# RobustFieldAutonomyLab/DRL_graph_exploration

Hardware: AMD Instinct MI355X
Metric: env-steps/sec (256 parallel envs, ~64-node graphs) (higher is better)
Workload: dtype f64; 1 GPU; configs[1]: 256 envs/GPU, 40x40 map (V=1600), 100 landmarks, belief update at ~59-node graphs (P=37.0 poses, L=22.2 landmarks, M=188 factors) from a device snapshot; envs_per_gpu=256, map_size=40, num_landmarks=100, parallelism=env-sharded x1

## Files before the change

### drl_graph_exploration_amd/_lib.py

```python
import ctypes as C
import os

from .config import DrlgxConfig

_HERE = os.path.dirname(os.path.abspath(__file__))
_PATH = os.environ.get("DRLGX_LIB_DEV", os.path.join(_HERE, "libdrlgx.so"))
_lib = None

N_TIMERS = 8


class DrlgxError(RuntimeError):
    pass


class CsrCache(C.Structure):
    _fields_ = [(n, C.c_void_p) for n in ("deg", "selfw", "ax", "ptr_dst", "end_dst", "ptr_src", "end_src", "nbr_dst", "nbr_src", "wn_dst",
                                          "wn_src")]
    NODE_WORDS = dict(deg=1, selfw=1, ax=8, ptr_dst=1, end_dst=1, ptr_src=1, end_src=1)
    EDGE_WORDS = dict(nbr_dst=1, nbr_src=1, wn_dst=1, wn_src=1)


def lib_path():
    return _PATH


SYMBOLS = [
    "drlgx_create", "drlgx_destroy", "drlgx_set_stream", "drlgx_synchronize", "drlgx_strerror", "drlgx_last_error",
    "drlgx_status_host", "drlgx_status_fetch_host", "drlgx_reset_host", "drlgx_step", "drlgx_utility", "drlgx_uncertainty_em", "drlgx_explored", "drlgx_metrics", "drlgx_cov_array",
    "drlgx_stage_reset_host", "drlgx_stage_set_prior_information_host", "drlgx_stage_set_prior_pose_host", "drlgx_stage_move", "drlgx_stage_measure", "drlgx_stage_add_measurements", "drlgx_stage_optimize",
    "drlgx_stage_update_map", "drlgx_set_planner_parameter", "drlgx_set_fixed_landmarks_host", "drlgx_fm2_update", "drlgx_fm2_update_steps", "drlgx_em_cost", "drlgx_em_cost_steps", "drlgx_set_dubins_leaf_scoring", "drlgx_em_plan_leaves", "drlgx_og_cost", "drlgx_set_sampler_parameter", "drlgx_set_sampler_obstacles", "drlgx_set_dubins_library_host", "drlgx_dubins_library", "drlgx_set_dubins_prefilter", "drlgx_em_plan", "drlgx_rrt_plan", "drlgx_step_plan", "drlgx_step_plans", "drlgx_step_plans_traced",
    "drlgx_line_plan", "drlgx_lookahead", "drlgx_lookahead_bounded", "drlgx_graph_capacity", "drlgx_graph", "drlgx_get_counts_host", "drlgx_counts",
    "drlgx_get_poses_host", "drlgx_get_landmarks_host", "drlgx_get_cov_traces_host", "drlgx_vm_shape",
    "drlgx_get_virtual_map_host", "drlgx_get_ground_truth_host", "drlgx_get_adjacency_host", "drlgx_get_factors_host",
    "drlgx_get_landmark_order_host", "drlgx_snapshot", "drlgx_restore", "drlgx_timing_enable",
    "drlgx_timing_read_host", "drlgx_debug_phase_clocks_host", "drlgx_debug_gemm_tile_rows", "drlgx_debug_map_form", "drlgx_debug_map_compact_ok", "drlgx_debug_disc_cells_bound", "drlgx_inc_stats_host", "drlgx_gcn_workspace_bytes", "drlgx_gcn_forward", "drlgx_gcn_forward_batched", "drlgx_gcn_backward",
    "drlgx_replay_collate", "drlgx_replay_collate_pair", "drlgx_dqn_targets", "drlgx_dqn_loss_grad", "drlgx_dqn_arena_bytes", "drlgx_dqn_arena_views", "drlgx_dqn_prepare", "drlgx_dqn_forward_backward", "drlgx_replay_cache_csr", "drlgx_gcn_collate_csr", "drlgx_gcn_forward_prebuilt", "drlgx_adam_step", "drlgx_adam_step_scaled", "drlgx_normalise_rewards",
    "drlgx_segment_softmax", "drlgx_segment_softmax_backward", "drlgx_mean_pool", "drlgx_mean_pool_backward",
    "drlgx_ggnn_workspace_bytes", "drlgx_ggnn_forward", "drlgx_ggnn_backward",
    "drlgx_greedy_plans",
    "drlgx_set_env_obstacles", "drlgx_obstacle_flags", "drlgx_follow_plans",
    "drlgx_unet_workspace_bytes", "drlgx_unet_forward", "drlgx_unet_backward", "drlgx_unet_topk", "drlgx_unet_augment_filter", "drlgx_unet_kept_nodes",
]


def lib():
    global _lib
    if _lib is not None:
        return _lib
    import torch
    if not os.path.exists(_PATH):
        raise DrlgxError(
            "libdrlgx.so not found at %s — build it with `python -c 'import __graft_entry__ as g; g.build()'` "
            "(hipcc --offload-arch=gfx950); there is no CPU fallback." % _PATH)
    L = C.CDLL(_PATH)
    vp, ip, dp = C.c_void_p, C.POINTER(C.c_int32), C.POINTER(C.c_double)
    L.drlgx_create.argtypes = [C.POINTER(DrlgxConfig), C.c_int, C.c_int, C.c_int, C.POINTER(vp)]
    L.drlgx_destroy.argtypes = [vp]
    L.drlgx_set_stream.argtypes = [vp, vp]
    L.drlgx_synchronize.argtypes = [vp]
    L.drlgx_strerror.restype = C.c_char_p
    L.drlgx_strerror.argtypes = [C.c_int]
    L.drlgx_last_error.restype = C.c_char_p
    L.drlgx_last_error.argtypes = [vp]
    L.drlgx_status_host.argtypes = [vp]
    L.drlgx_status_fetch_host.argtypes = [vp, vp, C.c_size_t, vp]
    L.drlgx_reset_host.argtypes = [vp, C.c_int, ip, C.POINTER(C.c_uint32), dp]
    L.drlgx_step.argtypes = [vp, vp, vp]
    L.drlgx_step_plan.argtypes = [vp, vp, vp, C.c_int, C.c_int]
    L.drlgx_step_plans.argtypes = [vp, vp, vp, C.c_int, C.c_int]
    L.drlgx_step_plans_traced.argtypes = [vp, vp, vp, C.c_int, C.c_double, C.c_double, C.c_int, vp, vp]
    L.drlgx_greedy_plans.argtypes = [vp, C.c_int, vp, C.c_int] + [vp] * 5 + [C.c_int, C.c_int, vp, vp, vp]
    if os.environ.get("DRLGX_LIB_DEV") is None or hasattr(L, "drlgx_follow_plans"):
        L.drlgx_set_env_obstacles.argtypes = [vp, C.c_int]
        L.drlgx_obstacle_flags.argtypes = [vp, vp]
        L.drlgx_follow_plans.argtypes = [vp, vp, vp, vp, vp, C.c_int, dp, C.c_double, C.c_double, C.c_int, vp, vp, vp, vp]
    L.drlgx_stage_reset_host.argtypes =[vp, C.c_int, ip, C.POINTER(C.c_uint32), dp]
    L.drlgx_stage_set_prior_information_host.argtypes = [vp, C.c_int, dp]
    L.drlgx_stage_set_prior_pose_host.argtypes = [vp, C.c_int, dp]
    L.drlgx_stage_move.argtypes = [vp, vp, vp]
    L.drlgx_stage_measure.argtypes = [vp, vp, vp, vp, vp]
    L.drlgx_stage_add_measurements.argtypes = [vp, vp, vp, vp, vp]
    L.drlgx_stage_optimize.argtypes = [vp, vp]
    L.drlgx_stage_update_map.argtypes = [vp, vp, C.c_int]
    L.drlgx_set_planner_parameter.argtypes = [vp, C.c_double, C.c_double, C.c_double, C.c_double, C.c_double, C.c_int]
    L.drlgx_set_fixed_landmarks_host.argtypes = [vp, C.c_int, dp]
    L.drlgx_fm2_update.argtypes = [vp, C.c_int, vp, vp, vp, vp, C.c_int, vp]
    L.drlgx_em_cost.argtypes = [vp, C.c_int, vp, vp, vp, C.c_int, vp, vp, vp]
    if os.environ.get("DRLGX_LIB_DEV") is None or hasattr(L, "drlgx_em_cost_steps"):
        L.drlgx_fm2_update_steps.argtypes = [vp, C.c_int, vp, vp, vp, vp, vp, C.c_int, vp]
        L.drlgx_em_cost_steps.argtypes = [vp, C.c_int, vp, vp, vp, vp, vp, C.c_int, vp, vp, vp]
        L.drlgx_set_dubins_leaf_scoring.argtypes = [vp, C.c_int]
        L.drlgx_em_plan_leaves.argtypes = [vp, C.c_int, ip, ip, vp, vp, vp, vp, vp, vp]
    L.drlgx_og_cost.argtypes = [vp, C.c_int, vp, vp, vp, vp, vp, vp]
    L.drlgx_set_sampler_parameter.argtypes = [vp, C.c_double, C.c_double, C.c_int]
    L.drlgx_set_sampler_obstacles.argtypes = [vp, C.c_int]
    L.drlgx_set_dubins_library_host.argtypes = [vp, dp]
    L.drlgx_dubins_library.argtypes = [vp, C.c_int, ip, dp, dp, dp, ip]
    L.drlgx_set_dubins_prefilter.argtypes = [vp, C.c_int]
    L.drlgx_em_plan.argtypes = [vp, C.c_int, vp, vp, C.c_int, C.c_int] + [vp] * 8
    L.drlgx_rrt_plan.argtypes = [vp, C.c_int, vp, vp, vp, vp, C.c_int] + [vp] * 6
    L.drlgx_utility.argtypes = [vp, vp, vp]
    L.drlgx_uncertainty_em.argtypes = [vp, C.c_int, vp]
    L.drlgx_explored.argtypes = [vp, vp]
    L.drlgx_metrics.argtypes = [vp, C.c_double, vp]
    L.drlgx_cov_array.argtypes = [vp, vp, vp]
    L.drlgx_line_plan.argtypes = [vp, C.c_int, vp, vp, vp, vp]
    L.drlgx_lookahead.argtypes = [vp, C.c_int, vp, vp, vp, vp]
    L.drlgx_lookahead_bounded.argtypes = [vp, C.c_int, vp, vp, vp, C.c_int, vp]
    L.drlgx_graph_capacity.argtypes = [vp, ip, ip, ip]
    L.drlgx_graph.argtypes = [vp] + [vp] * 8
    L.drlgx_get_counts_host.argtypes = [vp, C.c_int, ip]
    L.drlgx_counts.argtypes = [vp, vp]
    L.drlgx_get_poses_host.argtypes = [vp, C.c_int, dp, dp]
    L.drlgx_get_landmarks_host.argtypes = [vp, C.c_int, ip, dp, dp]
    L.drlgx_get_cov_traces_host.argtypes = [vp, C.c_int, dp, dp]
    L.drlgx_vm_shape.argtypes = [vp, ip, ip]
    L.drlgx_get_virtual_map_host.argtypes = [vp, C.c_int, dp, dp, dp, C.POINTER(C.c_uint8)]
    L.drlgx_get_ground_truth_host.argtypes = [vp, C.c_int, dp, dp]
    L.drlgx_get_adjacency_host.argtypes = [vp, C.c_int, dp, dp]
    L.drlgx_get_factors_host.argtypes = [vp, C.c_int, ip, ip, dp, dp]
    L.drlgx_get_landmark_order_host.argtypes = [vp, ip]
    L.drlgx_snapshot.argtypes = [vp, C.c_int]
    L.drlgx_restore.argtypes = [vp, C.c_int]
    L.drlgx_timing_enable.argtypes = [vp, C.c_int]
    L.drlgx_timing_read_host.argtypes = [vp, dp, C.POINTER(C.c_int64)]
    L.drlgx_debug_phase_clocks_host.argtypes = [vp, C.c_int, C.POINTER(C.c_int64)]
    L.drlgx_debug_gemm_tile_rows.argtypes = [C.c_int, C.c_int, C.c_int, C.c_int]
    L.drlgx_debug_map_form.argtypes = [C.c_int]
    L.drlgx_debug_map_compact_ok.argtypes = [vp, C.c_int]
    L.drlgx_debug_disc_cells_bound.argtypes = [C.c_double]
    L.drlgx_inc_stats_host.argtypes = [vp, C.POINTER(C.c_int64), C.c_int]
    L.drlgx_gcn_workspace_bytes.restype = C.c_size_t
    L.drlgx_gcn_workspace_bytes.argtypes = [C.c_int, C.c_int, C.c_int, C.c_int]
    L.drlgx_gcn_forward.argtypes = [vp] + [C.c_int] * 5 + [vp] * 12
    L.drlgx_gcn_backward.argtypes = [vp] + [C.c_int] * 5 + [vp] * 15
    L.drlgx_ggnn_workspace_bytes.restype = C.c_size_t
    L.drlgx_ggnn_workspace_bytes.argtypes = [C.c_int] * 5
    L.drlgx_ggnn_forward.argtypes = [vp] + [C.c_int] * 6 + [vp] * 13 + [C.c_int, vp, vp, C.c_int]
    L.drlgx_ggnn_backward.argtypes = [vp] + [C.c_int] * 6 + [vp] * 17
    L.drlgx_unet_workspace_bytes.restype = C.c_size_t
    L.drlgx_unet_workspace_bytes.argtypes = [C.c_int] * 6 + [C.c_double, C.c_int]
    L.drlgx_unet_forward.argtypes = [vp] + [C.c_int] * 5 + [C.c_double, C.c_int] + [vp] * 3 + [C.POINTER(vp)] + [vp] * 3 + [C.c_size_t, C.c_int, vp, vp,
                                                                                                                       C.c_int]
    L.drlgx_unet_backward.argtypes = [vp] + [C.c_int] * 5 + [C.c_double, C.c_int] + [vp] * 3 + [C.POINTER(vp), vp, vp, C.POINTER(vp), vp, C.c_size_t,
                                                                                                C.c_int, C.c_int]
    L.drlgx_unet_kept_nodes.argtypes = [vp] + [C.c_int] * 4 + [C.c_double, C.c_int, vp, C.c_size_t, C.c_int, C.c_int, C.c_int, vp, C.POINTER(C.c_int)]
    L.drlgx_unet_topk.argtypes = [vp, C.c_int, C.c_int, vp, vp, C.c_double, vp, vp, vp, vp]
    L.drlgx_unet_augment_filter.argtypes = [vp, C.c_int, C.c_int, vp, vp, C.c_int, vp, vp, C.c_int, vp, vp, vp, C.c_int64, vp, vp, vp]
    L.drlgx_replay_collate.argtypes = [vp, C.c_int, vp, vp, C.c_int, vp, C.c_int64, vp, vp, vp, C.c_int64, vp, vp, vp, vp, vp, vp]
    L.drlgx_replay_collate_pair.argtypes = [vp, C.c_int, vp, vp, C.c_int, vp, C.c_int64, vp, vp, vp, C.c_int64, vp, vp, vp, vp, vp, vp, vp]
    L.drlgx_gcn_forward_batched.argtypes = [vp] + [C.c_int] * 5 + [vp] * 12 + [C.c_int, vp, vp, C.c_int]
    L.drlgx_dqn_targets.argtypes = [vp, C.c_int, vp, vp, vp, C.c_double, C.c_int64, vp, vp]
    L.drlgx_dqn_loss_grad.argtypes = [vp, C.c_int, vp, vp, vp, C.c_double, vp, vp]
    i64 = C.c_int64
    L.drlgx_dqn_arena_bytes.restype = C.c_size_t
    L.drlgx_dqn_arena_bytes.argtypes = [C.c_int, i64, i64, i64, C.c_int, C.c_int, C.c_int]
    L.drlgx_dqn_arena_views.argtypes = [vp, C.c_int, i64, i64, i64, C.c_int, C.c_int, C.c_int, C.POINTER(vp)]
    L.drlgx_dqn_prepare.argtypes = [vp, C.c_int, vp, vp, vp, C.c_int, vp, i64, vp, vp, i64, i64, i64, vp, vp, C.c_double, vp, i64, i64, i64,
                                    C.c_int, C.c_int, C.POINTER(CsrCache)]
    L.drlgx_dqn_forward_backward.argtypes = [vp, C.c_int, i64, i64, C.c_int, C.c_int, C.c_int, C.c_int, C.POINTER(vp), vp, C.c_double,
                                             C.POINTER(vp), vp, i64, i64, i64, C.c_int]
    L.drlgx_replay_cache_csr.argtypes = [vp, C.c_int, vp, vp, C.c_int, vp, C.c_int, vp, i64, vp, C.POINTER(CsrCache)]
    L.drlgx_gcn_collate_csr.argtypes = [vp, C.c_int, vp, C.POINTER(CsrCache), C.c_int, C.c_int, C.c_int, C.c_int, vp, vp, vp, vp, vp, vp]
    L.drlgx_gcn_forward_prebuilt.argtypes = [vp] + [C.c_int] * 5 + [vp] * 9
    L.drlgx_normalise_rewards.argtypes = [vp, C.c_int, vp, vp, vp, vp, vp]
    L.drlgx_segment_softmax.argtypes = [vp, C.c_int, vp, vp, vp, vp]
    L.drlgx_segment_softmax_backward.argtypes = [vp, C.c_int, vp, vp, vp, vp, vp]
    L.drlgx_mean_pool.argtypes = [vp, C.c_int, vp, vp, C.c_int, vp]
    L.drlgx_mean_pool_backward.argtypes = [vp, C.c_int, vp, vp, C.c_int, vp]
    L.drlgx_adam_step.argtypes = [vp, C.c_int, C.POINTER(vp), C.POINTER(vp), C.POINTER(vp), C.POINTER(vp), C.POINTER(C.c_int64),
                                  C.c_double, C.c_double, C.c_double, C.c_double, C.c_int64, C.c_double]
    L.drlgx_adam_step_scaled.argtypes = [vp, C.c_int, C.POINTER(vp), C.POINTER(vp), C.POINTER(vp), C.POINTER(vp), C.POINTER(C.c_int64),
                                  C.c_double, C.c_double, C.c_double, C.c_double, C.c_int64, C.c_double, C.c_double]
    _lib = L
    return L


def stream_ptr(device):
    import torch
    idx = device.index if isinstance(device, torch.device) else device
    if idx is None:
        idx = torch.cuda.current_device()
    return torch._C._cuda_getCurrentRawStream(idx)


def check(rc, handle=None):
    if rc != 0:
        L = lib()
        msg = L.drlgx_strerror(rc).decode()
        if handle is not None:
            extra = L.drlgx_last_error(handle).decode()
            if extra:
                msg += " (" + extra + ")"
        raise DrlgxError("drlgx error %d: %s" % (rc, msg))
```

### drl_graph_exploration_amd/csrc/drlgx_dev.h

```cpp
#pragma once
#include <hip/hip_runtime.h>
#include <stdint.h>

#include "../../include/drlgx.h"
#include "map_carve.h"

#define DRLGX_MT_N 624
#define DRLGX_MT_STRIDE 626
#define DRLGX_CNT_STRIDE 8
#define DRLGX_RED_STRIDE 8
#define DRLGX_PRIOR_STRIDE 16

enum { C_P = 0, C_L = 1, C_M = 2, C_STEP = 3, C_ISAM = 4, C_NEWP = 5, C_NEWL = 6, C_FLAG = 7 };
enum { R_UTR = 0, R_KNOWN = 1, R_EXPL = 2, R_UDET = 3, R_UWTR = 4, R_DIST = 5, R_OBS = 6, R_LATCH = 7 };

struct DrlgxState {
  drlgx_config cfg;
  int n_envs, n_inst, n_roll;
  int P_max, L_max, M_max, LG, V, Vu, rows, cols, A_max;
  int win;
  int disc_cells;
  int count_explored;
  double lo_free, lo_occ, lo_min, lo_max, occ_thresh;
  int bbox_noop;
// ... 13 lines not shown
  double *gt_lm;
  const double *fixed_lm;
  int n_fixed;
  int *parent;
  uint32_t *mt;
  double *nrm_saved;
  int *nrm_has;
  int *cnt;
  double *th_pose;
  double *d_pose;
  double *th_lm;
  double *d_lm;
  int *lm_key;
  int *key_slot;
  double *prior;
  double *odo;
  int *meas_pose;
  int *meas_lm;
  double *meas_br;
  double *est_pose;
  double *est_lm;
  double *pose_info;
  double *lm_info;
  double *pose_tr;
  double *lm_tr;
  double *vm_prob;
  double *vm_info;
  uint8_t *vm_upd;
  double *vm_tr;
  double *red;
  double *slam_ws;
  size_t slam_ws_stride;
  int *slam_iws;
  size_t slam_iws_stride;
  int *status;
  double *jc;
  size_t jc_stride;
  int jc_ld;
  double *jd;
  int *jc_meta;
  unsigned long long *inc_stats;
  long long *prof;
  int prof_block;
  const DrlgxState *self_dev;
};

typedef const __attribute__((address_space(4))) DrlgxState *DrlgxStateConst;
__device__ __forceinline__ void drlgx_warm_state(DrlgxStateConst Sp) {
  static_assert(sizeof(DrlgxState) <= 14 * 64, "drlgx_warm_state touches fourteen lines");
  const unsigned long long sp = reinterpret_cast<unsigned long long>(Sp);
  unsigned int w0, w1, w2, w3, w4, w5, w6, w7, w8, w9, w10, w11, w12, w13;
  asm volatile("s_load_dword %0, %14, 0x0\n\ts_load_dword %1, %14, 0x40\n\ts_load_dword %2, %14, 0x80\n\t"
               "s_load_dword %3, %14, 0xc0\n\ts_load_dword %4, %14, 0x100\n\ts_load_dword %5, %14, 0x140\n\t"
               "s_load_dword %6, %14, 0x180\n\ts_load_dword %7, %14, 0x1c0\n\ts_load_dword %8, %14, 0x200\n\t"
               "s_load_dword %9, %14, 0x240\n\ts_load_dword %10, %14, 0x280\n\ts_load_dword %11, %14, 0x2c0\n\t"
               "s_load_dword %12, %14, 0x300\n\ts_load_dword %13, %14, 0x340\n\t"
               "s_waitcnt lgkmcnt(0)"
               : "=s"(w0), "=s"(w1), "=s"(w2), "=s"(w3), "=s"(w4), "=s"(w5), "=s"(w6), "=s"(w7), "=s"(w8), "=s"(w9), "=s"(w10), "=s"(w11),
                 "=s"(w12), "=s"(w13)
               : "s"(sp));
}

#define DRLGX_KS_PARAM DrlgxStateConst S_
#define DRLGX_KS_REF (*(const DrlgxState *)S_)
#define DRLGX_KS_ARG(S) ((DrlgxStateConst)(S).self_dev)

#define DRLGX_PROF(S, slot)                                                        \
  do {                                                                             \
    if ((S).prof && threadIdx.x == 0 && blockIdx.x == (S).prof_block) (S).prof[slot] = wall_clock64(); \
  } while (0)

__device__ __forceinline__ int drlgx_bid() {
  int b = blockIdx.x;
  asm volatile("" : "+v"(b));
  return __builtin_amdgcn_readfirstlane(b);
}

__device__ __forceinline__ int drlgx_tid() {
  int t = threadIdx.x;
  asm volatile("" : "+v"(t));
  return t;
}

struct LaunchSel {
  int base;
  int n;
  const uint8_t *active;
  const int32_t *n_act;
  int act_idx;
  int map_last_only = 0;
  int pcap = 0;
  int skip_map = 0;
  const unsigned char *simlog = nullptr;
  size_t simlog_roll = 0;
  int simlog_act = 0;
  int vm_from = -1;
  __host__ __device__ __forceinline__ int cap(int P_max) const { return pcap > 0 && pcap < P_max ? pcap : P_max; }
  __device__ __forceinline__ bool map_on(int i) const {
    return !(map_last_only && n_act) || act_idx == n_act[i] - 1;
  }
  __device__ __forceinline__ bool on(int i) const {
    if (active && !active[i]) return false;
    if (n_act && act_idx >= n_act[i]) return false;
    return true;
  }
};

struct Pose {
  double x, y, c, s;
};
struct P2 {
  double x, y;
};

__device__ __forceinline__ void rot_from_cos_sin(double c, double s, double &oc, double &os) {
  if (fabs(c * c + s * s - 1.0) > 1e-9) {
    double n = sqrt(c * c + s * s);
    c /= n;
    s /= n;
  }
  oc = c;
  os = s;
}
__device__ __forceinline__ Pose make_pose(double x, double y, double th) { return Pose{x, y, cos(th), sin(th)}; }
__device__ __forceinline__ double theta_of(const Pose &p) { return atan2(p.s, p.c); }
__device__ __forceinline__ Pose compose(const Pose &a, const Pose &b) {
  Pose r;
  rot_from_cos_sin(a.c * b.c - a.s * b.s, a.s * b.c + a.c * b.s, r.c, r.s);
  r.x = a.x + (a.c * b.x - a.s * b.y);
  r.y = a.y + (a.s * b.x + a.c * b.y);
  return r;
}
__device__ __forceinline__ Pose between(const Pose &p1, const Pose &p2, double *H1) {
  double c = p1.c * p2.c + p1.s * p2.s, s = -p1.s * p2.c + p1.c * p2.s;
  Pose r;
  rot_from_cos_sin(c, s, r.c, r.s);
  double dx = p2.x - p1.x, dy = p2.y - p1.y;
  r.x = p1.c * dx + p1.s * dy;
  r.y = -p1.s * dx + p1.c * dy;
  if (H1) {
    double dt1 = -p2.s * dx + p2.c * dy;
    double dt2 = -p2.c * dx - p2.s * dy;
    H1[0] = -r.c; H1[1] = -r.s; H1[2] = dt1;
    H1[3] = r.s;  H1[4] = -r.c; H1[5] = dt2;
    H1[6] = 0;    H1[7] = 0;    H1[8] = -1;
  }
  return r;
}
__device__ __forceinline__ P2 transform_to(const Pose &p, const P2 &pt) {
  double dx = pt.x - p.x, dy = pt.y - p.y;
  return P2{p.c * dx + p.s * dy, -p.s * dx + p.c * dy};
}
__device__ __forceinline__ P2 transform_from(const Pose &p, const P2 &q) {
  return P2{p.c * q.x - p.s * q.y + p.x, p.s * q.x + p.c * q.y + p.y};
}
template <bool JAC>
__device__ __forceinline__ double bearing_of(const Pose &p, const P2 &pt, double *Hx, double *Hl) {
  P2 d = transform_to(p, pt);
  double d2 = d.x * d.x + d.y * d.y, n = sqrt(d2);
  if (fabs(n) > 1e-5) {
    if (JAC) {
      double a = -d.y / d2, b = d.x / d2;
      Hx[0] = a * -1.0;
      Hx[1] = b * -1.0;
      Hx[2] = a * d.y + b * -d.x;
      Hl[0] = a * p.c + b * -p.s;
// ... 295 lines not shown
    const double x = 2.0 * mt_canonical_words(mt_peek(s, w), mt_peek(s, w + 1)) - 1.0;
    const double y = 2.0 * mt_canonical_words(mt_peek(s, w + 2), mt_peek(s, w + 3)) - 1.0;
    const double r2 = x * x + y * y;
    const bool acc = !(r2 > 1.0 || r2 == 0.0);
    const unsigned long long m = __ballot(acc);
    const int rank = __popcll(m & ((1ull << lane) - 1ull));
    const int j = have + rank;
    const int i0 = offset + 2 * j;
    if (acc && j < Np && i0 + 1 >= skip) {
      const double mult = sqrt(-2 * log(r2) / r2);
      if (i0 >= skip) out[i0 - skip] = y * mult;
      out[i0 + 1 - skip] = x * mult;
    }
    const int A = __popcll(m);
    if (have + A >= Np) {
      const unsigned long long last = __ballot(acc && rank == Np - have - 1);
      const int t = __ffsll((long long)last) - 1;
      s.cons += 4u * (uint32_t)(t + 1);
      have = Np;
    } else {
      s.cons += 256u;
      have += A;
    }
  }
  wave_lds_sync();
  if (R & 1) {
    ns.saved = out[count - skip];
    ns.has = 1;
  }
}
__device__ inline double rng_normal(MtStream &s, NormalState &ns, double m, double sd, int lane) {
  return normal01(s, ns, lane) * sd + m;
}
__device__ inline double rng_uniform_real(MtStream &s, double lo, double hi, int lane) {
  return (hi - lo) * mt_canonical(s, lane) + lo;
}

inline void drlgx_ensure_lds_attr(bool (&done)[32], const void *const *fns, int n, int bytes) {
  int dev = 0;
  if (hipGetDevice(&dev) != hipSuccess || dev < 0 || dev >= 32) dev = 0;
  if (done[dev]) return;
  for (int i = 0; i < n; ++i) (void)hipFuncSetAttribute(fns[i], hipFuncAttributeMaxDynamicSharedMemorySize, bytes);
  done[dev] = true;
}

__host__ __device__ inline size_t drlgx_sim_lds_bytes(int LG, int P_max) {
  size_t b = (size_t)2 * DRLGX_MT_STRIDE * 4 + (size_t)(2 * LG + 2) * 8 + (size_t)LG * 4 + 16;
  b = ((b + 7) & ~(size_t)7) + (size_t)2 * LG * 8;
  if (P_max <= 64) b = b > kmap::MapCarve::pose_tables_bytes(P_max) + 32 ? b : kmap::MapCarve::pose_tables_bytes(P_max) + 32;
  return (b + 31) & ~(size_t)31;
}

struct DrlgxField;
enum DrlgxSimLaunch { DRLGX_SIM_RESET, DRLGX_SIM_STEP, DRLGX_SIM_STEP_OBS, DRLGX_SIM_STAGE, DRLGX_SIM_PRESIM };
constexpr size_t kSimLdsLimit = 64 * 1024;
size_t drlgx_sim_launch_lds(DrlgxSimLaunch which, int LG, int n_measure = 1, size_t *dyn_out = nullptr);
void drlgx_launch_reset(const DrlgxState &S, hipStream_t st, int n, const int32_t *env_ids_dev, const uint32_t *seeds_dev,
                        const double *start_dev, int first_measure = 1);
void drlgx_launch_sim_stage(const DrlgxState &S, hipStream_t st, LaunchSel sel, const double *odom, int mode, int32_t *keys,
                            double *br, int32_t *count);
void drlgx_launch_add_measurements(const DrlgxState &S, hipStream_t st, LaunchSel sel, const int32_t *keys, const double *br,
                                   const int32_t *count);
size_t drlgx_simlog_entry_bytes(const DrlgxState &S);
void drlgx_launch_presim(const DrlgxState &S, hipStream_t st, LaunchSel sel, const double *odom, int odom_stride, int n_measure, int a_end,
                         unsigned char *simlog, size_t simlog_roll, int simlog_act);
void drlgx_launch_sim(const DrlgxState &S, hipStream_t st, LaunchSel sel, const double *odom, int odom_stride,
                      int n_measure);
void drlgx_launch_sim_obs(const DrlgxState &S, hipStream_t st, LaunchSel sel, const double *odom, int odom_stride);
void drlgx_launch_slam(const DrlgxState &S, hipStream_t st, LaunchSel sel, int p_bound);
size_t drlgx_map_lds_bytes(const DrlgxState &S, int *chunk_out, int pcap = 0);
bool drlgx_step_fusable(const DrlgxState &S, int p_bound);
bool drlgx_step_arrow_fusable(const DrlgxState &S);
void drlgx_launch_step_arrow(const DrlgxState &S, hipStream_t st, LaunchSel sel, const double *odom, int odom_stride, int n_measure);
void drlgx_launch_step(const DrlgxState &S, hipStream_t st, LaunchSel sel, const double *odom, int odom_stride, int n_measure);
void drlgx_launch_step_loop(const DrlgxState &S, hipStream_t st, LaunchSel sel, const double *odom, int odom_stride, int n_measure, int a_end);
void drlgx_launch_step_arrow_loop(const DrlgxState &S, hipStream_t st, LaunchSel sel, const double *odom, int odom_stride, int n_measure, int a_end);
void drlgx_launch_map(const DrlgxState &S, hipStream_t st, LaunchSel sel, int rebuild);
bool drlgx_map_two_per_cu(const DrlgxState &S, int p_bound);
bool drlgx_map_compact_ok(const DrlgxState &S, int p_bound);
void drlgx_launch_copy(const DrlgxField *fields_dev, int n_fields, hipStream_t st, int n, const int32_t *src,
                       const int32_t *dst, int src_off, int dst_off, int skip_mask,
                       const int *cnt = nullptr,
                       const DrlgxState *panel = nullptr,
                       int only_cls = -1);
void drlgx_launch_rebase(const DrlgxState &S, hipStream_t st, int base0, int n);
inline size_t drlgx_fetch_head_bytes(int n_envs) { return ((size_t)(n_envs + 1) * sizeof(int) + 15) & ~(size_t)15; }
void drlgx_launch_fetch_pack(const DrlgxState &S, hipStream_t st, const void *src, size_t bytes, void *out);
void drlgx_launch_fix_rollouts(const DrlgxState &S, hipStream_t st, int n_cand, const int32_t *cand_env, int roll0);
void drlgx_launch_rewards(const DrlgxState &S, hipStream_t st, int n_cand, const int32_t *cand_env, int roll0,
                          double *rewards);
void drlgx_launch_utility(const DrlgxState &S, hipStream_t st, const double *dist, double *out, int mode);
void drlgx_launch_fm2_prior(const DrlgxState &S, hipStream_t st, const int32_t *env_ids, int n_env, double *sig, size_t sig_stride,
                            int n_max);
size_t drlgx_fm2_scratch_doubles(const DrlgxState &S, int nm_max);
void drlgx_launch_fm2_check(const DrlgxState &S, hipStream_t st, int n_cand, const int32_t *cand_env, const double *actions,
                            const int32_t *n_actions, const uint8_t *core, int nm_max, int *flag);
void drlgx_launch_fm2_update(const DrlgxState &S, hipStream_t st, int c0, int nc, const int32_t *cand_env, const int32_t *env_slot,
                             const double *actions, const int32_t *n_actions, const uint8_t *core, const double *sig, size_t sig_stride,
                             double *scratch, size_t scratch_stride, int *iscratch, int nm_max, double *cov_out, int out_stride,
                             int32_t *n_out);
size_t drlgx_em_lds_bytes(const DrlgxState &S);
void drlgx_launch_em_cost(const DrlgxState &S, hipStream_t st, int nc, const int32_t *cand_env, const double *actions,
                          const int32_t *n_actions, const uint8_t *core, const double *distance, const double *cov, int cov_stride,
                          int algorithm, double *unc_out, double *cost_out, double *info_out);
size_t drlgx_og_lds_bytes(const DrlgxState &S);
void drlgx_launch_og_check(const DrlgxState &S, hipStream_t st, int n_cand, const int32_t *cand_env, const int32_t *n_actions, int *flag);
void drlgx_launch_og_cost(const DrlgxState &S, hipStream_t st, int nc, const int32_t *cand_env, const double *actions,
                          const int32_t *n_actions, double *ent_out, double *cost_out, double *prob_out);
struct DrlgxDubins {
  const double *end_x, *end_y, *v, *w;
  const int *num_steps;
  int n, max_steps;
  double dt, tol, reach;
  double *pose;
};
struct DrlgxTreeArgs {
  int n_sel;
  const int32_t *env_sel;
  const int32_t *halton_start;
  int cap;
  int mode;
  double max_nodes;
  double safe_distance;
  const int32_t *goal_key;
  const double *goal_xy;
  double *act;
  int *link;
  int *leaf;
  int *meta;
  int *flag;
  double *nodes_out;
  int32_t *n_nodes_out, *result_out, *halton_next_out;
  DrlgxDubins lib;
};
size_t drlgx_em_tree_lds_bytes(int cap);
void drlgx_launch_em_tree(const DrlgxState &S, hipStream_t st, DrlgxTreeArgs args, bool obstacles, bool dubins);
void drlgx_launch_em_leaves_dubins(hipStream_t st, int n_sel, const int32_t *env_sel, int cap, int A_max, double angle_weight,
                                   const double *act, const int *link, const int *leaf, const int *meta, const DrlgxDubins &lib,
                                   int per_tree_row, int32_t *cand_env, double *actions, int32_t *n_actions, uint8_t *core,
                                   double *distance);
void drlgx_launch_em_leaves(hipStream_t st, int n_sel, const int32_t *env_sel, int cap, int A_max, const double *act, const int *link,
                            const int *leaf, const int *meta, int per_tree_row, int32_t *cand_env, double *actions, int32_t *n_actions);
void drlgx_launch_em_pick(hipStream_t st, int n_sel, int A_max, const int *meta, const double *cost, const double *actions,
                          const int32_t *n_actions, double *plan_out, int32_t *n_actions_out, double *cost_out, int32_t *n_leaves_out);
void drlgx_launch_metrics(const DrlgxState &S, hipStream_t st, double sigma0, double *out);
void drlgx_launch_plan_record(const DrlgxState &S, hipStream_t st, double sigma0, int a, int32_t *n_actions, double done_explored,
                              int max_steps, double *trace, int32_t *done);
void drlgx_launch_follow_select(const DrlgxState &S, hipStream_t st, const double *plan, const int32_t *n_actions, const int32_t *result,
                                const uint8_t *active, int steps, const double *fallback, double *act, int32_t *n_exec, int32_t *stop);
void drlgx_launch_follow_record(const DrlgxState &S, hipStream_t st, double sigma0, int a, const double *act, int32_t *n_exec, int obstacles,
                                double done_explored, int max_steps, double *trace, int32_t *done, int32_t *stop);
void drlgx_launch_obstacle_flags(const DrlgxState &S, hipStream_t st, uint8_t *out);
void drlgx_launch_cov_array(const DrlgxState &S, hipStream_t st, double *length, double *angle);
void drlgx_launch_line_plan(const DrlgxState &S, hipStream_t st, int n_cand, const int32_t *cand_env, const double *goal,
                            double *actions, int32_t *n_actions);
bool drlgx_slam_in_lds(int P_max, int L_max, int M_max);
bool drlgx_slam_capacity_ok(int P_max, int L_max, int M_max);
size_t drlgx_slam_ws_doubles(int P_max, int L_max, int M_max);
bool drlgx_graph_capacity_ok(int P_max, int L_max, int V);
void drlgx_launch_graph(const DrlgxState &S, hipStream_t st, int *gi, int gi_stride, int32_t *node_off, int32_t *edge_off,
                        float *x, int64_t *edge_index, float *edge_attr, int32_t *n_frontier, double *frontier_xy,
                        int32_t *nearest_node, int max_frontier);
```

### drl_graph_exploration_amd/csrc/drlgx_engine.cpp

```cpp
#include <hip/hip_runtime.h>

#include <algorithm>
#include <chrono>
#include <cmath>
#include <cstdio>
#include <cstring>
#include <functional>
#include <string>
#include <unordered_map>
#include <cstdlib>
#include <vector>

#include "drlgx_dev.h"
#include "drlgx_fields.h"

#define HIPCHK(e, call)                                                                       \
  do {                                                                                        \
    hipError_t _r = (call);                                                                   \
    if (_r != hipSuccess) {                                                                   \
      (e)->last_error = std::string(#call) + ": " + hipGetErrorString(_r);                    \
      return DRLGX_E_HIP;                                                                     \
    }                                                                                         \
  } while (0)

// ... 470 lines not shown
    std::unordered_map<unsigned, int> m;
    for (int i = 0; i < cfg->num_landmarks; ++i) m.emplace((unsigned)i, i);
    for (const auto &kv : m) e->lm_order.push_back((int)kv.first);
    if (e->lm_order.empty()) e->lm_order.push_back(0);
  }
  TRY(upload_table(e, &S.sweep_b, sweep));
  TRY(upload_table(e, &S.lm_order, e->lm_order));
  TRY(upload_table(e, &S.lo_pv, lo_pv));
  TRY(alloc_fields(e));
  S.slam_ws_stride = drlgx_slam_ws_doubles(S.P_max, S.L_max, S.M_max);
  S.slam_iws_stride = 2;
  TRY(dev_alloc(e, &S.slam_ws, S.slam_ws_stride * (size_t)S.n_inst));
  TRY(dev_alloc(e, &S.slam_iws, S.slam_iws_stride * (size_t)S.n_inst));
  TRY(alloc_panels(e));
  TRY(alloc_staging(e));
  HIPCHK(e, hipStreamSynchronize(e->stream));
  return DRLGX_OK;
}
#undef TRY

extern "C" {

const char *drlgx_strerror(int code) {
  switch (code) {
    case DRLGX_OK: return "ok";
    case DRLGX_E_INVALID: return "invalid argument";
    case DRLGX_E_NODEVICE: return "no HIP device";
    case DRLGX_E_CAPACITY: return "instance capacity exceeded (max_poses / max_landmarks / max_factors / max_actions)";
    case DRLGX_E_HIP: return "HIP runtime error";
    case DRLGX_E_NUMERIC: return "indeterminate linear system in the SLAM solve";
    default: return "unknown error";
  }
}

const char *drlgx_last_error(const drlgx_engine *e) {
  if (e) return e->last_error.c_str();
  return g_create_error.empty() ? "null engine" : g_create_error.c_str();
}

int drlgx_create(const drlgx_config *cfg, int n_envs, int n_rollouts, int device, drlgx_engine **out) {
  if (!out) return DRLGX_E_INVALID;
  g_create_error.clear();
  int r = check_config(cfg, n_envs, n_rollouts);
  if (r) return r;
  int ndev = 0;
  if (hipGetDeviceCount(&ndev) != hipSuccess || ndev <= 0 || device < 0 || device >= ndev) return DRLGX_E_NODEVICE;
  drlgx_engine *e = new drlgx_engine();
  e->device = device;
  if (hipSetDevice(device) != hipSuccess) {
    delete e;
    return DRLGX_E_NODEVICE;
  }
  if (hipStreamCreateWithFlags(&e->own_stream, hipStreamNonBlocking) != hipSuccess) {
    delete e;
    return DRLGX_E_NODEVICE;
  }
  e->stream = e->own_stream;
  DrlgxState &S = e->S;
  S.cfg = *cfg;
  S.n_envs = n_envs;
  S.n_roll = n_rollouts;
  if ((r = build_engine(e)) != DRLGX_OK) {
    g_create_error = e->last_error;
    drlgx_destroy(e);
    return r;
  }
  state_sync(e);
  *out = e;
  return DRLGX_OK;
}

static void state_sync(drlgx_engine *e) {
  if (!e->state_dev || memcmp(e->state_shadow, &e->S, sizeof(DrlgxState)) == 0) return;
  (void)hipStreamSynchronize(e->stream);
  (void)hipMemcpy(e->state_dev, &e->S, sizeof(DrlgxState), hipMemcpyHostToDevice);
  memcpy(e->state_shadow, &e->S, sizeof(DrlgxState));
}

static int snapshot_base(const drlgx_engine *e, int slot) { return 2 * e->S.n_envs + e->S.n_roll + slot * e->S.n_envs; }

static void settle(drlgx_engine *e) {
  if (e->owed_slot < 0) return;
  drlgx_launch_copy(e->fields_dev, (int)e->fields.size(), e->stream, e->S.n_envs, nullptr, nullptr, snapshot_base(e, e->owed_slot), 0, 0,
                    nullptr, nullptr, 1);
  e->owed_slot = -1;
}

int drlgx_destroy(drlgx_engine *e) {
  DRLGX_ENTER_OWING(e);
  if (!e) return DRLGX_E_INVALID;
  hipDeviceSynchronize();
  for (void *p : e->allocs) hipFree(p);
  for (auto &sp : e->spans) {
    hipEventDestroy(sp.a);
    hipEventDestroy(sp.b);
  }
  for (auto ev : e->free_events) hipEventDestroy(ev);
  if (e->sync_event) hipEventDestroy(e->sync_event);
  if (e->fetch_dev) hipFree(e->fetch_dev);
  if (e->fetch_host) hipHostFree(e->fetch_host);
  if (e->own_stream) hipStreamDestroy(e->own_stream);
  delete e;
  return DRLGX_OK;
}

int drlgx_set_stream(drlgx_engine *e, void *hip_stream) {
  DRLGX_ENTER_OWING(e);
  if (!e) return DRLGX_E_INVALID;
  hipStream_t s = (hip_stream == reinterpret_cast<void *>(-1)) ? e->own_stream : reinterpret_cast<hipStream_t>(hip_stream);
  if (s == e->stream) return DRLGX_OK;
  hipStreamSynchronize(e->stream);
  e->stream = s;
  return DRLGX_OK;
}

int drlgx_synchronize(drlgx_engine *e) {
  DRLGX_ENTER_OWING(e);
  if (!e) return DRLGX_E_INVALID;
  HIPCHK(e, hipStreamSynchronize(e->stream));
  return DRLGX_OK;
}

static int max_bound(const drlgx_engine *e) {
  if (e->by_capacity) return e->S.P_max;
  int m = 1;
  for (int v : e->pbound) m = std::max(m, v);
  return m;
}

static void advance_pbound(drlgx_engine *e, int k) {
  for (int &v : e->pbound) v = std::min(v + k, e->S.P_max);
}

static hipError_t stream_wait(drlgx_engine *e) {
  if (!e->spin_sync) return hipStreamSynchronize(e->stream);
  if (!e->sync_event && hipEventCreateWithFlags(&e->sync_event, hipEventDisableTiming) != hipSuccess) {
    (void)hipGetLastError();
    e->spin_sync = false;
    return hipStreamSynchronize(e->stream);
  }
  hipError_t r = hipEventRecord(e->sync_event, e->stream);
  if (r != hipSuccess) return r;
  const auto t0 = std::chrono::steady_clock::now();
  for (int polls = 0; (r = hipEventQuery(e->sync_event)) == hipErrorNotReady; ++polls) {
    if ((polls & 63) == 63 && std::chrono::steady_clock::now() - t0 > std::chrono::microseconds(5000)) return hipStreamSynchronize(e->stream);
  }
  return r;
}

static int status_fetch(drlgx_engine *e, const void *src_dev, size_t bytes, void *dst_host) {
  const size_t head = drlgx_fetch_head_bytes(e->S.n_envs), total = head + ((bytes + 15) & ~(size_t)15);
  if (total > e->fetch_cap) {
    HIPCHK(e, hipStreamSynchronize(e->stream));
    if (e->fetch_dev) (void)hipFree(e->fetch_dev);
    if (e->fetch_host) (void)hipHostFree(e->fetch_host);
    e->fetch_dev = e->fetch_host = nullptr;
    e->fetch_cap = 0;
    const size_t cap = std::max<size_t>(2 * total, 1 << 16);
    HIPCHK(e, hipMalloc(reinterpret_cast<void **>(&e->fetch_dev), cap));
    HIPCHK(e, hipHostMalloc(reinterpret_cast<void **>(&e->fetch_host), cap, hipHostMallocDefault));
    e->fetch_cap = cap;
  }
  drlgx_launch_fetch_pack(e->S, e->stream, src_dev, bytes, e->fetch_dev);
  HIPCHK(e, hipMemcpyAsync(e->fetch_host, e->fetch_dev, head + bytes, hipMemcpyDeviceToHost, e->stream));
  HIPCHK(e, stream_wait(e));
  const int32_t *h = reinterpret_cast<const int32_t *>(e->fetch_host);
  for (int i = 0; i < e->S.n_envs; ++i) e->pbound[i] = std::min(std::max((int)h[1 + i], 1), e->S.P_max);
// ... 998 lines not shown
  if (r) return r;
  const DrlgxState &S = e->S;
  const int L = c[1], M = c[2];
  std::vector<int> keys(L), mp(M), ml(M);
  std::vector<double> br((size_t)M * 2);
  if ((r = fetch(e, keys.data(), S.lm_key + (size_t)inst * S.L_max, (size_t)L * 4))) return r;
  if ((r = fetch(e, mp.data(), S.meas_pose + (size_t)inst * S.M_max, (size_t)M * 4))) return r;
  if ((r = fetch(e, ml.data(), S.meas_lm + (size_t)inst * S.M_max, (size_t)M * 4))) return r;
  if ((r = fetch(e, br.data(), S.meas_br + (size_t)inst * S.M_max * 2, (size_t)M * 16))) return r;
  HIPCHK(e, hipStreamSynchronize(e->stream));
  for (int m = 0; m < M; ++m) {
    if (pose) pose[m] = mp[m];
    if (key) key[m] = keys[ml[m]];
    if (bearing) bearing[m] = br[2 * m];
    if (range) range[m] = br[2 * m + 1];
  }
  return DRLGX_OK;
}

int drlgx_get_adjacency_host(drlgx_engine *e, int inst, double *adjacency, double *features) {
  DRLGX_ENTER(e);
  int32_t c[5];
  int r = drlgx_get_counts_host(e, inst, c);
  if (r) return r;
  const DrlgxState &S = e->S;
  const int P = c[0], L = c[1], M = c[2], N = P + L;
  std::vector<int> k, ord;
  if ((r = sorted_slots(e, inst, L, k, ord))) return r;
  std::vector<int> node_of_slot(L);
  for (int n = 0; n < L; ++n) node_of_slot[ord[n]] = n;
  std::vector<int> mp(M), ml(M);
  std::vector<double> br((size_t)M * 2), odo((size_t)P * 4), lt(L), pt(P);
  if ((r = fetch(e, mp.data(), S.meas_pose + (size_t)inst * S.M_max, (size_t)M * 4))) return r;
  if ((r = fetch(e, ml.data(), S.meas_lm + (size_t)inst * S.M_max, (size_t)M * 4))) return r;
  if ((r = fetch(e, br.data(), S.meas_br + (size_t)inst * S.M_max * 2, (size_t)M * 16))) return r;
  if ((r = fetch(e, odo.data(), S.odo + (size_t)inst * S.P_max * 4, (size_t)P * 32))) return r;
  if ((r = fetch(e, lt.data(), S.lm_tr + (size_t)inst * S.L_max, (size_t)L * 8))) return r;
  if ((r = fetch(e, pt.data(), S.pose_tr + (size_t)inst * S.P_max, (size_t)P * 8))) return r;
  HIPCHK(e, hipStreamSynchronize(e->stream));
  if (adjacency) std::fill(adjacency, adjacency + (size_t)N * N, 0.0);
  if (features) std::fill(features, features + N, 0.0);
  for (int i = 0; i + 1 < P; ++i) {
    double d = std::sqrt(std::pow(odo[4 * i], 2) + std::pow(odo[4 * i + 1], 2)) + 0.001;
    int a = L + i, b = L + i + 1;
    if (adjacency) adjacency[(size_t)a * N + b] = adjacency[(size_t)b * N + a] = d;
    if (features) {
      features[a] = pt[i];
      features[b] = pt[i + 1];
    }
  }
  for (int m = 0; m < M; ++m) {
    int a = L + mp[m], b = node_of_slot[ml[m]];
    if (adjacency) adjacency[(size_t)a * N + b] = adjacency[(size_t)b * N + a] = br[2 * m + 1];
    if (features) {
      features[a] = pt[mp[m]];
      features[b] = lt[ml[m]];
    }
  }
  return DRLGX_OK;
}

int drlgx_get_landmark_order_host(const drlgx_engine *e, int32_t *order) {
  if (!e || !order) return DRLGX_E_INVALID;
  for (int i = 0; i < e->S.cfg.num_landmarks; ++i) order[i] = e->lm_order[i];
  return DRLGX_OK;
}

int drlgx_snapshot(drlgx_engine *e, int slot) {
  DRLGX_ENTER(e);
  if (!e || slot < 0 || slot >= e->S.cfg.max_snapshots) return DRLGX_E_INVALID;
  const DrlgxState &S = e->S;
  ScopedTimer t(e, 3);
  drlgx_launch_copy(e->fields_dev, (int)e->fields.size(), e->stream, S.n_envs, nullptr, nullptr, 0, snapshot_base(e, slot), 0, e->S.cnt, &S);
  e->snap_pbound[slot] = e->pbound;
  return check_launch(e);
}

int drlgx_restore(drlgx_engine *e, int slot) {
  DRLGX_ENTER_OWING(e);
  if (!e || slot < 0 || slot >= e->S.cfg.max_snapshots) return DRLGX_E_INVALID;
  const DrlgxState &S = e->S;
  ScopedTimer t(e, 3);
  drlgx_launch_copy(e->fields_dev, (int)e->fields.size(), e->stream, S.n_envs, nullptr, nullptr, snapshot_base(e, slot), 0,
                    e->restore_eager ? 0 : 1, e->S.cnt, &S);
  e->owed_slot = e->restore_eager ? -1 : slot;
  e->pbound = e->snap_pbound[slot];
  return check_launch(e);
}

int drlgx_debug_phase_clocks_host(drlgx_engine *e, int arm, int64_t out[64]) {
  DRLGX_ENTER(e);
  if (!e) return DRLGX_E_INVALID;
  HIPCHK(e, hipStreamSynchronize(e->stream));
  e->S.prof_block = (arm >> 8) & 0xffff;
  if (out && e->S.prof)
    HIPCHK(e, hipMemcpy(out, e->S.prof + ((arm & 4) ? 0 : ((arm & 2) ? 64 : 0)), ((arm & 4) ? 1024 : 64) * sizeof(long long), hipMemcpyDeviceToHost));
  if (arm && !e->S.prof) {
    long long *p = nullptr;
    int r = dev_alloc(e, &p, 1024);
    if (r) return r;
    HIPCHK(e, hipStreamSynchronize(e->stream));
    e->S.prof = p;
  } else if (!arm) {
    e->S.prof = nullptr;
  }
  return DRLGX_OK;
}

int drlgx_inc_stats_host(drlgx_engine *e, int64_t out[2], int reset) {
  DRLGX_ENTER_OWING(e);
  if (!e || !out) return DRLGX_E_INVALID;
  out[0] = out[1] = -1;
  if (!e->S.inc_stats) return DRLGX_OK;
  unsigned long long v[2] = {0, 0};
  HIPCHK(e, hipMemcpyAsync(v, e->S.inc_stats, sizeof(v), hipMemcpyDeviceToHost, e->stream));
  if (reset) HIPCHK(e, hipMemsetAsync(e->S.inc_stats, 0, sizeof(v), e->stream));
  HIPCHK(e, hipStreamSynchronize(e->stream));
  out[0] = (int64_t)v[0];
  out[1] = (int64_t)v[1];
  return DRLGX_OK;
}

int drlgx_timing_enable(drlgx_engine *e, int on) {
  DRLGX_ENTER_OWING(e);
  if (!e) return DRLGX_E_INVALID;
  e->timing = on != 0;
  e->per_stage = on == 2;
  return DRLGX_OK;
}

int drlgx_timing_read_host(drlgx_engine *e, double ms[DRLGX_N_TIMERS], int64_t launches[DRLGX_N_TIMERS]) {
  DRLGX_ENTER_OWING(e);
  if (!e) return DRLGX_E_INVALID;
  HIPCHK(e, hipStreamSynchronize(e->stream));
  for (auto &sp : e->spans) {
    float t = 0;
    if (hipEventElapsedTime(&t, sp.a, sp.b) == hipSuccess && sp.id >= 0 && sp.id < DRLGX_N_TIMERS) {
      e->t_ms[sp.id] += t;
      e->t_n[sp.id] += 1;
    }
    e->free_events.push_back(sp.a);
    e->free_events.push_back(sp.b);
  }
  e->spans.clear();
  for (int i = 0; i < DRLGX_N_TIMERS; ++i) {
    if (ms) ms[i] = e->t_ms[i];
    if (launches) launches[i] = e->t_n[i];
    e->t_ms[i] = 0;
    e->t_n[i] = 0;
  }
  return DRLGX_OK;
}

}
```

### drl_graph_exploration_amd/csrc/k_inc.hip

```cpp

#pragma once
#include <type_traits>
#include "k_slam_common.hip"
namespace kslam {
#pragma clang fp contract(on)

constexpr int IYS = 18;
constexpr int INF = 64;
constexpr int kStreamKB = 512;
constexpr int ISNT = 4;

__device__ __forceinline__ int *inc_meta(const DrlgxState &S, int inst) { return S.jc_meta + (size_t)inst * 4; }

__device__ __forceinline__ bool inc_precheck(const DrlgxState &S, int inst, int P_after, int tid, int *scratch, int meta0 = -1, int meta1 = 0,
                                             int isam = 0) {
  if (!S.jc) return false;
  const int *meta = inc_meta(S, inst);
  const int *cnt = S.cnt + (size_t)inst * DRLGX_CNT_STRIDE;
  if (meta0 < 0) {
    meta0 = meta[0];
    meta1 = meta[1];
    isam = cnt[C_ISAM];
  }
  if (meta0 != 1 || meta1 + 1 != P_after || P_after < 2) return false;
// ... 22 lines not shown
    if constexpr (kDist == 16) {
      const auto p = __builtin_amdgcn_permlane16_swap(w[h], w[h], false, false);
      w[h] = ((threadIdx.x >> 4) & 1) ? p[0] : p[1];
    } else {
      const auto p = __builtin_amdgcn_permlane32_swap(w[h], w[h], false, false);
      w[h] = ((threadIdx.x >> 5) & 1) ? p[0] : p[1];
    }
  }
  return __longlong_as_double(((long long)w[1] << 32) | w[0]);
}

template <int kShift>
__device__ __forceinline__ double row_shr_f64(double v) {
  const long long b = __double_as_longlong(v);
  const int lo = __builtin_amdgcn_update_dpp(0, (int)b, 0x110 + kShift, 0xf, 0xf, true);
  const int hi = __builtin_amdgcn_update_dpp(0, (int)(b >> 32), 0x110 + kShift, 0xf, 0xf, true);
  return __longlong_as_double(((long long)hi << 32) | (unsigned int)lo);
}

constexpr int INEW = 12;
struct IncCtx {
  int inst, P, pn, pp, L0, M0, Lcap, n1, n1p, a0, ldw;
  int *fre, *fnew, *fslot, *ictl;
  double *fq, *recs, *gs, *vvec, *wks, *thp, *thl, *dl, *Dl, *Y, *Yh, *cwl;
  bool wide;
  int snt, yrows;
  double *yt, *wim, *jt, *svv;
};
__device__ __forceinline__ bool inc_plan(const DrlgxState &S, int inst, int P, int lds_bytes, size_t smem_off, IncCtx &x, bool &lds_panel, int pc,
                                         int L0_known = -1, int M0_known = -1) {
  extern __shared__ __attribute__((aligned(16))) unsigned char smem_raw[];
  const int *meta = inc_meta(S, inst);
  x.inst = inst; x.P = P; x.pn = P - 1; x.pp = P - 2;
  x.L0 = L0_known >= 0 ? L0_known : meta[2];
  x.M0 = L0_known >= 0 ? M0_known : meta[3];
  x.Lcap = min(S.L_max, x.L0 + INEW);
  x.n1 = 3 * P + 2 * x.L0; x.n1p = (x.n1 + 15) & ~15;
  x.a0 = 3 + 2 * x.L0;
  x.ldw = (3 + 2 * x.Lcap + 31) & ~31;
  const int ncap = max(3 * P + 2 * x.Lcap, x.n1p);
  size_t plan_off = drlgx_sim_lds_bytes(S.LG, pc);
  if ((3 * P + 1 + 15) / 16 > kDenseTiles && 2 * S.L_max + 1 > 16 * 8) plan_off = 0;
  if (smem_off > plan_off) plan_off = smem_off;
  size_t off = (smem_off + 15) & ~(size_t)15;
  const size_t off0 = off;
  auto take = [&](size_t bytes) { unsigned char *q = smem_raw + off; off += (bytes + 15) & ~(size_t)15; return q; };
  x.fre = reinterpret_cast<int *>(take(INF * 4));
  x.fnew = reinterpret_cast<int *>(take(INF * 4));
  x.fslot = reinterpret_cast<int *>(take(INF * 4));
  x.ictl = reinterpret_cast<int *>(take(16));
  x.fq = reinterpret_cast<double *>(take(32 * 8));
  x.recs = reinterpret_cast<double *>(take(INF * REC * 8));
  x.gs = reinterpret_cast<double *>(take(INEW * 12 * 8));
  x.vvec = reinterpret_cast<double *>(take(32 * 8));
  x.wks = reinterpret_cast<double *>(take(5 * 16 * IYS * 8));
  x.thp = reinterpret_cast<double *>(take((size_t)P * 4 * 8));
  x.thl = reinterpret_cast<double *>(take((size_t)x.Lcap * 2 * 8));
  x.dl = reinterpret_cast<double *>(take((size_t)ncap * 8));
  x.Dl = reinterpret_cast<double *>(take((size_t)P * 6 * 8));
  x.Y = reinterpret_cast<double *>(take((size_t)(x.n1p + 1) * IYS * 8));
  x.cwl = reinterpret_cast<double *>(smem_raw + off);
  const size_t fixed = ((plan_off + 15) & ~(size_t)15) + (off - off0);
  if (fixed > (size_t)lds_bytes) return false;
  lds_panel = fixed + (size_t)ncap * x.ldw * 8 <= (size_t)lds_bytes;
  const size_t pan = lds_panel ? (size_t)ncap * x.ldw * 8 : 0, yh = (size_t)(x.n1p + 1) * IYS * 8;
  x.Yh = x.cwl + pan / 8;
  x.wide = fixed + pan + yh <= (size_t)lds_bytes;
  x.snt = 0;
  if (!lds_panel && (3 * P + 1 + 15) / 16 > kDenseTiles) {
    x.yrows = x.a0 + 1;
    const size_t y_off = (size_t)(reinterpret_cast<unsigned char *>(x.Y) - smem_raw);
    const size_t avail = (size_t)lds_bytes - (((plan_off + 15) & ~(size_t)15) + (y_off - off0));
    for (int t = ISNT; t >= 1 && !x.snt; --t)
      if ((size_t)t * x.yrows * IYS * 8 + (size_t)max(0, t * t - 5) * 16 * IYS * 8 + (size_t)16 * t * 8 * 8 + 64 * 8 <= avail) x.snt = t;
    x.yt = x.Y;
    x.wim = x.yt + (size_t)x.snt * x.yrows * IYS;
    x.jt = x.wim + (size_t)max(0, x.snt * x.snt - 5) * 16 * IYS;
    x.svv = x.jt + (size_t)16 * x.snt * 8;
  }
  return true;
}

template <bool kLds, bool kSub>
__device__ __forceinline__ void inc_pre(const DrlgxState &S, const IncCtx &x, int tid, const double *odom3, SubBarrier sb) {
  const int ft = kSub ? tid - 64 : tid, fn = kSub ? kThreads - 64 : kThreads, lane = tid & 63;
  auto bar = [&]() {
    if constexpr (kSub) sb.sync(lane);
    else __syncthreads();
  };
  const int inst = x.inst, P = x.P, pn = x.pn, pp = x.pp, L0 = x.L0, n1 = x.n1, a0 = x.a0;
  double *gpan = S.jc + (size_t)inst * S.jc_stride;
  auto growp = [&](int q) -> double * { return gpan + (size_t)(q < 3 * P ? q : q + 3 * (S.P_max - P)) * S.jc_ld; };
  auto rowp = [&](int q) -> double * {
    if constexpr (kLds) return x.cwl + (size_t)q * x.ldw;
    else return gpan + (size_t)(q < 3 * P ? q : q + 3 * (S.P_max - P)) * S.jc_ld;
  };
  const double *th_pose = S.th_pose + (size_t)inst * S.P_max * 4;
  const double *th_lm = S.th_lm + (size_t)inst * S.L_max * 2;
  const double *d_pose = S.d_pose + (size_t)inst * S.P_max * 3;
  const double *d_lm = S.d_lm + (size_t)inst * S.L_max * 2;
  const double *jd = S.jd + (size_t)inst * S.P_max * 6;
  if (S.prof && blockIdx.x == S.prof_block && ft == 0) S.prof[0] = wall_clock64();
  if (ft < 4) x.ictl[ft] = 0;
  if (ft == fn - 1) {
    const double *t1 = th_pose + 4 * pp;
    Pose p1{t1[0], t1[1], t1[2], t1[3]}, p2, om;
    if constexpr (kSub) {
      om = make_pose(odom3[0], odom3[1], odom3[2]);
      const double *ep = S.est_pose + ((size_t)inst * S.P_max + pp) * 4;
      p2 = compose(Pose{ep[0], ep[1], ep[2], ep[3]}, om);
    } else {
      const double *t2 = th_pose + 4 * pn, *oo = S.odo + ((size_t)inst * S.P_max + pp) * 4;
      p2 = Pose{t2[0], t2[1], t2[2], t2[3]};
      om = Pose{oo[0], oo[1], oo[2], oo[3]};
    }
    double H1[9];
    const Pose hx = between(p1, p2, H1);
    const Pose h = between(om, hx, nullptr);
    const double e0 = h.x, e1 = h.y, e2 = theta_of(h);
    double *fq = x.fq;
    for (int k = 0; k < 9; ++k) fq[k] = -H1[k];
    fq[9] = -(h.c * e0 - h.s * e1);
    fq[10] = -(h.s * e0 + h.c * e1);
    fq[11] = -e2;
    x.thp[4 * pn] = p2.x; x.thp[4 * pn + 1] = p2.y; x.thp[4 * pn + 2] = p2.c; x.thp[4 * pn + 3] = p2.s;
  }
  for (int e = ft; e < 4 * pn; e += fn) x.thp[e] = th_pose[e];
  for (int e = ft; e < 2 * L0; e += fn) x.thl[e] = th_lm[e];
  for (int e = ft; e < 3 * pn; e += fn) x.dl[e] = d_pose[e];
  for (int e = ft; e < 2 * L0; e += fn) x.dl[3 * P + e] = d_lm[e];
  for (int e = ft; e < 6 * pn; e += fn) x.Dl[e] = jd[e];
  if constexpr (kLds) {
    const int npair = (a0 + 1) >> 1, nr = n1 - 3;
    const int cp0 = ft & 31, r0 = ft >> 5, rs = fn >> 5;
    for (int cp = cp0; cp < npair; cp += 32)
      for (int qq = r0; qq < nr; qq += 4 * rs) {
        const int q0 = qq, q1 = qq + rs, q2 = qq + 2 * rs, q3 = qq + 3 * rs;
        auto src = [&](int q) { const int c = min(q, nr - 1); return reinterpret_cast<const double2 *>(growp(c < 3 * pn ? c : c + 3))[cp]; };
        const double2 v0 = src(q0), v1 = src(q1), v2 = src(q2), v3 = src(q3);
        auto dst = [&](int q, const double2 &v) { if (q < nr) reinterpret_cast<double2 *>(rowp(q < 3 * pn ? q : q + 3))[cp] = v; };
        dst(q0, v0); dst(q1, v1); dst(q2, v2); dst(q3, v3);
      }
  }
  for (int e = ft; e < (x.n1p + 1 - n1) * IYS; e += fn) {
    x.Y[(size_t)n1 * IYS + e] = 0.0;
    if (x.wide) x.Yh[(size_t)n1 * IYS + e] = 0.0;
  }
  bar();
  if (S.prof && blockIdx.x == S.prof_block && ft == 0) S.prof[1] = wall_clock64();
  const double *fq = x.fq;
  {
    const double f00 = fq[0], f01 = fq[1], f02 = fq[2], f10 = fq[3], f11 = fq[4], f12 = fq[5], f20 = fq[6], f21 = fq[7], f22 = fq[8];
    for (int qq = ft; qq < n1 - 3; qq += fn) {
      const int q = qq < 3 * pn ? qq : qq + 3;
      double *r = rowp(q);
      const double t0 = r[0], t1 = r[1], t2 = r[2];
      r[0] = f00 * t0 + f01 * t1 + f02 * t2;
      r[1] = f10 * t0 + f11 * t1 + f12 * t2;
      r[2] = f20 * t0 + f21 * t1 + f22 * t2;
    }
  }
  bar();
  for (int e = ft; e < 3 * a0; e += fn) {
    const int r = e / a0, c = e - r * a0;
    double v = fq[3 * r] * rowp(3 * pp)[c] + fq[3 * r + 1] * rowp(3 * pp + 1)[c] + fq[3 * r + 2] * rowp(3 * pp + 2)[c];
    if (c == r) v += 1.0 / (c < 2 ? S.w_trans : S.w_rot);
    rowp(3 * pn + r)[c] = v;
  }
  if (ft < 3) x.dl[3 * pn + ft] = fq[3 * ft] * x.dl[3 * pp] + fq[3 * ft + 1] * x.dl[3 * pp + 1] + fq[3 * ft + 2] * x.dl[3 * pp + 2] + fq[9 + ft];
  if (S.prof && blockIdx.x == S.prof_block && ft == 0) S.prof[2] = wall_clock64();
}

template <bool kLds, int kSNT = ISNT>
__device__ __forceinline__ bool inc_post(const DrlgxState &S, const IncCtx &x, int L, int M, const SimBox &box, int tid,
                                         double *hand = nullptr, int hand_cap = 0) {
  const int lane = tid & 63, wave = tid >> 6, lc = lane & 15, lr = lane >> 4;
  const int inst = x.inst, P = x.P, pn = x.pn, L0 = x.L0, M0 = x.M0, n1 = x.n1, n1p = x.n1p, a0 = x.a0;
  int *meta = inc_meta(S, inst);
  const int nf = M - M0, nn = L - L0;
  const int n = 3 * P + 2 * L, a = 3 + 2 * L;
  int *fre = x.fre, *fnew = x.fnew, *fslot = x.fslot, *ictl = x.ictl;
  double *recs = x.recs, *gs = x.gs, *vvec = x.vvec, *wks = x.wks, *thp = x.thp, *thl = x.thl, *dl = x.dl, *Dl = x.Dl, *Y = x.Y;
  double *gpan = S.jc + (size_t)inst * S.jc_stride;
  auto growp = [&](int q) -> double * { return gpan + (size_t)(q < 3 * P ? q : q + 3 * (S.P_max - P)) * S.jc_ld; };
  auto rowp = [&](int q) -> double * {
    if constexpr (kLds) return x.cwl + (size_t)q * x.ldw;
    else return gpan + (size_t)(q < 3 * P ? q : q + 3 * (S.P_max - P)) * S.jc_ld;
  };
  int *cnt = S.cnt + (size_t)inst * DRLGX_CNT_STRIDE;
  double *d_pose = S.d_pose + (size_t)inst * S.P_max * 3;
  double *d_lm = S.d_lm + (size_t)inst * S.L_max * 2;
  double *jd = S.jd + (size_t)inst * S.P_max * 6;
  const bool feasible = nf >= 0 && nf <= INF && nn >= 0 && nn <= nf && L <= x.Lcap;
  const int *slot_src = box.br ? box.slot : S.meas_lm + (size_t)inst * S.M_max + M0;
  const double *br_src = box.br ? box.br : S.meas_br + ((size_t)inst * S.M_max + M0) * 2;
  const double *nl_src = box.br ? box.lm : S.th_lm + ((size_t)inst * S.L_max + L0) * 2;
  if (feasible && tid < 64) {
    const bool have = tid < nf;
    const int slot = have ? slot_src[tid] : -1;
    if (have) fslot[tid] = slot;
    bool bad = have && (slot < 0 || slot >= L);
    if (have && !box.br) bad |= S.meas_pose[(size_t)inst * S.M_max + M0 + tid] != pn;
    for (int t = 0; t < nf; ++t) {
      const int st = __builtin_amdgcn_readlane(slot, t);
      bad |= have && t < tid && st == slot;
    }
    const bool re = have && slot < L0, nw = have && slot >= L0;
    const unsigned long long mre = __ballot(re), mnw = __ballot(nw);
    if (re) fre[__popcll(mre & ((1ull << lane) - 1ull))] = tid;
    if (nw && !bad) fnew[slot - L0] = tid;
    if ((__ballot(bad) || __popcll(mnw) != nn) && lane == 0) ictl[2] = 1;
    if (lane == 0) ictl[0] = __popcll(mre);
  }
  for (int e = tid - 64; e >= 0 && e < 2 * nn && feasible; e += kThreads - 64) thl[2 * L0 + e] = nl_src[e];
  __syncthreads();
  if (!feasible || ictl[2]) {
    if (!kLds && tid == 0) meta[0] = 0;
    return false;
  }
  const int n_re = ictl[0];
  if (tid < nf) linearize_br(thp + 4 * pn, thl + 2 * fslot[tid], br_src[2 * tid], br_src[2 * tid + 1], recs + (size_t)REC * tid);
  __syncthreads();
  DRLGX_PROF(S, 35);
  const double Rb = S.cfg.bearing_noise * S.cfg.bearing_noise, Rr = S.cfg.range_noise * S.cfg.range_noise;
  const int ntr = n1p >> 4, ntc = (a0 + 15) >> 4;
  auto batch = [&](int b0, int nb, auto wide_tag) {
    constexpr bool kWide = decltype(wide_tag)::value;
    const int k = 2 * nb, kD = kWide ? k - 16 : 0;
    double *Yh = x.Yh;
    {
      constexpr int FS = kWide ? 16 : 8, RS = kThreads / FS;
      const int f = tid & (FS - 1);
      double j0 = 0, j1 = 0, j2 = 0, j3 = 0, j4 = 0, j5 = 0, l0c = 0, l1c = 0, l2c = 0, l3c = 0;
      int cl = 3;
      if (f < nb) {
        const int t = fre[b0 + f];
        const double *rc = recs + (size_t)REC * t;
        j0 = rc[0]; j1 = rc[1]; j2 = rc[2]; j3 = rc[3]; j4 = rc[4]; j5 = rc[5];
        l0c = rc[6]; l1c = rc[7]; l2c = rc[8]; l3c = rc[9];
        cl = 3 + 2 * fslot[t];
      }
      double *Yf = (kWide && f >= 8) ? Yh : Y;
      const int k0 = ks16(2 * (f & 7)), k1 = ks16(2 * (f & 7) + 1);
      for (int q0 = tid / FS; q0 < n1; q0 += 4 * RS) {
        double c0[4], c1[4], c2[4], l0[4], l1[4];
#pragma unroll
        for (int u = 0; u < 4; ++u) {
          const double *r = rowp(min(q0 + u * RS, n1 - 1));
          c0[u] = r[0]; c1[u] = r[1]; c2[u] = r[2]; l0[u] = r[cl]; l1[u] = r[cl + 1];
        }
#pragma unroll
        for (int u = 0; u < 4; ++u) {
          const int q = q0 + u * RS;
          if (q < n1) {
            Yf[(size_t)q * IYS + k0] = c0[u] * j0 + c1[u] * j1 + c2[u] * j2 + l0[u] * l0c + l1[u] * l1c;
            Yf[(size_t)q * IYS + k1] = c0[u] * j3 + c1[u] * j4 + c2[u] * j5 + l0[u] * l2c + l1[u] * l3c;
          }
        }
      }
    }
    __syncthreads();
    if (b0 == 0) DRLGX_PROF(S, 36);
    if (wave == 0) {
      auto tent = [&](int i, int j) -> double {
        const int t = fre[b0 + (i >> 1)], u = i & 1;
        const double *rc = recs + (size_t)REC * t;
        const double *Yj = (kWide && j >= 16) ? Yh : Y;
        const int col = ks16(j & 15);
        const double *yp = Yj + (size_t)(3 * pn) * IYS + col, *yl = Yj + (size_t)(3 * P + 2 * fslot[t]) * IYS + col;
        double sv = rc[3 * u] * yp[0] + rc[3 * u + 1] * yp[IYS] + rc[3 * u + 2] * yp[2 * IYS] + rc[6 + 2 * u] * yl[0] + rc[7 + 2 * u] * yl[IYS];
        if (i == j) sv += u ? Rr : Rb;
        return sv;
      };
      if (lane < (kWide ? 32 : 16)) {
        double v = 0.0;
        if (lane < k) {
          const int t = fre[b0 + (lane >> 1)], u = lane & 1;
          const double *rc = recs + (size_t)REC * t;
          const double *dp = dl + 3 * pn, *dq = dl + 3 * P + 2 * fslot[t];
          v = -rc[10 + u] - (rc[3 * u] * dp[0] + rc[3 * u + 1] * dp[1] + rc[3 * u + 2] * dp[2] + rc[6 + 2 * u] * dq[0] + rc[7 + 2 * u] * dq[1]);
        }
        vvec[(lane & 16) + ks16(lane & 15)] = v;
      }
      const int kA = kWide ? 16 : k;
      v4d d = {0.0, 0.0, 0.0, 0.0};
#pragma unroll
      for (int r = 0; r < 4; ++r) {
        const int i = lr + 4 * r, hi = max(i, lc), lo = min(i, lc);
        if (hi < kA) d[r] = tent(hi, lo);
      }
      const SweepCtx sx{0, lane, lc, lr, kA, 16, true, true, ictl + 1, nullptr};
      if constexpr (!kWide) {
        inv16_blk<true>(sx, kA, d);
        double *o = wks + lc * IYS + 4 * lr;
#pragma unroll
        for (int r = 0; r < 4; ++r) o[r] = (lc < k && lr + 4 * r < k) ? d[r] : 0.0;
      } else {
        v4d tb = {0.0, 0.0, 0.0, 0.0}, td = {0.0, 0.0, 0.0, 0.0};
#pragma unroll
        for (int r = 0; r < 4; ++r) {
          const int i = lr + 4 * r, hi = max(i, lc), lo = min(i, lc);
          if (lc < kD) tb[r] = tent(16 + lc, i);
          if (hi < kD) td[r] = tent(16 + hi, 16 + lo);
        }
        inv16_blk<false>(sx, 16, d);
        double a4[4] = {d[0], d[1], d[2], d[3]}, b4[4] = {tb[0], tb[1], tb[2], tb[3]};
        v4d xp = {0.0, 0.0, 0.0, 0.0};
        xp = mfma4(a4, b4, xp);
        double x4[4] = {xp[0], xp[1], xp[2], xp[3]};
        td = mfma4(b4, x4, td);
        const SweepCtx sd{0, lane, lc, lr, kD, 16, true, true, ictl + 1, nullptr};
        inv16_blk<true>(sd, kD, td);
        double *tsc = wks + 4 * 16 * IYS;
#pragma unroll
        for (int r = 0; r < 4; ++r) tsc[(lr + 4 * r) * IYS + ks16(lc)] = xp[r];
        wave_lds_sync();
        double xt4[4], s4[4];
        ld4(tsc + lc * IYS + 4 * lr, xt4);
#pragma unroll
        for (int r = 0; r < 4; ++r) s4[r] = (lc < kD && lr + 4 * r < kD) ? td[r] : 0.0;
        v4d w10 = {0.0, 0.0, 0.0, 0.0};
        w10 = mfma4(s4, xt4, w10);
        double w10a[4] = {w10[0], w10[1], w10[2], w10[3]};
        d = mfma4(w10a, xt4, d);
        double *o0 = wks + lc * IYS + 4 * lr, *o1 = o0 + 16 * IYS, *o3 = o0 + 3 * 16 * IYS;
#pragma unroll
        for (int r = 0; r < 4; ++r) {
          o0[r] = d[r];
          o1[r] = w10[r];
          o3[r] = s4[r];
          wks[2 * 16 * IYS + (lr + 4 * r) * IYS + ks16(lc)] = w10[r];
        }
      }
    }
    __syncthreads();
    if (b0 == 0) DRLGX_PROF(S, 37);
    if (wave < ntr) {
      const int npr = (a0 + 31) >> 5;
      const int nks = kWide ? 4 : (k + 3) >> 2;
      const int nks1 = kWide ? (kD + 3) >> 2 : 0;
      const int nun = ((ntr - wave + kWaves - 1) / kWaves) * npr;
      v4d aA0, aA1, aB0, aB1;
      double ua[4] = {0.0, 0.0, 0.0, 0.0}, ub[4] = {0.0, 0.0, 0.0, 0.0};
      auto loads = [&](int e, v4d &c0, v4d &c1) {
        const int it = e / npr, pr = e - it * npr, I = wave + kWaves * it;
#pragma unroll
        for (int r = 0; r < 4; ++r) {
          const double *rw = rowp(16 * I + lr + 4 * r) + 32 * pr + lc;
          c0[r] = rw[0];
          c1[r] = rw[16];
        }
      };
      auto unit = [&](int e, v4d &acc0, v4d &acc1) {
        const int it = e / npr, pr = e - it * npr, I = wave + kWaves * it;
        if (pr == 0) {
          double w4[4], yI[4], yH[4];
          ld4(wks + lc * IYS + 4 * lr, w4);
          ld4(Y + (size_t)(16 * I + lc) * IYS + 4 * lr, yI);
          v4d ut = {0.0, 0.0, 0.0, 0.0};
          ut = mfma4(w4, yI, ut);
          if constexpr (kWide) {
            ld4(Yh + (size_t)(16 * I + lc) * IYS + 4 * lr, yH);
            ld4(wks + 16 * IYS + lc * IYS + 4 * lr, w4);
            ut = mfma4(w4, yH, ut);
            v4d u2 = {0.0, 0.0, 0.0, 0.0};
            ld4(wks + 2 * 16 * IYS + lc * IYS + 4 * lr, w4);
            u2 = mfma4(w4, yI, u2);
            ld4(wks + 3 * 16 * IYS + lc * IYS + 4 * lr, w4);
            u2 = mfma4(w4, yH, u2);
            ub[0] = u2[0]; ub[1] = u2[1]; ub[2] = u2[2]; ub[3] = u2[3];
          }
          ua[0] = ut[0]; ua[1] = ut[1]; ua[2] = ut[2]; ua[3] = ut[3];
          const int q = 16 * I + lc;
          auto rowdot = [&](const double *vec, const double *vech) -> double {
            double y4[4];
            ld4(vec + 4 * lr, y4);
            double sdot = ua[0] * y4[0] + ua[1] * y4[1] + ua[2] * y4[2] + ua[3] * y4[3];
            if constexpr (kWide) {
              ld4(vech + 4 * lr, y4);
              sdot += ub[0] * y4[0] + ub[1] * y4[1] + ub[2] * y4[2] + ub[3] * y4[3];
            }
            sdot += rowgroup_xor<16>(sdot);
            sdot += rowgroup_xor<32>(sdot);
            return sdot;
          };
          const double sv = rowdot(vvec, vvec + 16);
          const bool prow = q < 3 * pn;
          const int qc = prow ? q : 0, pi = qc / 3, rp = qc - 3 * pi;
          const size_t o3 = (size_t)(3 * pi) * IYS;
          const double s0 = rowdot(Y + o3, Yh + o3), s1 = rowdot(Y + o3 + IYS, Yh + o3 + IYS), s2 = rowdot(Y + o3 + 2 * IYS, Yh + o3 + 2 * IYS);
          if (lr == 0 && q < n1) {
            dl[q] -= sv;
            if (prow) {
              double *D = Dl + 6 * pi + (rp * (rp + 1)) / 2;
              D[0] += s0;
              if (rp >= 1) D[1] += s1;
              if (rp >= 2) D[2] += s2;
            }
          }
        }
        {
          const int cA = 32 * pr + lc, cB = cA + 16;
          const int y0 = cA < 3 ? 3 * pn + cA : (cA < a0 ? 3 * P + cA - 3 : n1p);
          const int y1 = cB < a0 ? 3 * P + cB - 3 : n1p;
          double yJ0[4], yJ1[4];
          ld4(Y + (size_t)y0 * IYS + 4 * lr, yJ0);
          ld4(Y + (size_t)y1 * IYS + 4 * lr, yJ1);
#pragma unroll
          for (int ks = 0; ks < 4; ++ks)
            if (ks < nks) {
              acc0 = __builtin_amdgcn_mfma_f64_16x16x4f64(ua[ks], yJ0[ks], acc0, 0, 0, 0);
              acc1 = __builtin_amdgcn_mfma_f64_16x16x4f64(ua[ks], yJ1[ks], acc1, 0, 0, 0);
            }
          if constexpr (kWide) {
            ld4(Yh + (size_t)y0 * IYS + 4 * lr, yJ0);
            ld4(Yh + (size_t)y1 * IYS + 4 * lr, yJ1);
#pragma unroll
            for (int ks = 0; ks < 4; ++ks)
              if (ks < nks1) {
                acc0 = __builtin_amdgcn_mfma_f64_16x16x4f64(ub[ks], yJ0[ks], acc0, 0, 0, 0);
                acc1 = __builtin_amdgcn_mfma_f64_16x16x4f64(ub[ks], yJ1[ks], acc1, 0, 0, 0);
              }
          }
        }
#pragma unroll
        for (int r = 0; r < 4; ++r) {
          double *rw = rowp(16 * I + lr + 4 * r) + 32 * pr + lc;
          rw[0] = acc0[r];
          rw[16] = acc1[r];
        }
      };
      int e = 0;
      loads(0, aA0, aA1);
// ... 225 lines not shown
            }
          }
          sv += rowgroup_xor<16>(sv); sv += rowgroup_xor<32>(sv);
          so += rowgroup_xor<16>(so); so += rowgroup_xor<32>(so);
          s1 += rowgroup_xor<16>(s1); s1 += rowgroup_xor<32>(s1);
          s2 += rowgroup_xor<16>(s2); s2 += rowgroup_xor<32>(s2);
          if (lr == 0 && q >= 0) {
            dl[q] -= sv;
            if (q < 3 * pn) {
              const int pi = q / 3, rp = q - 3 * pi;
              double *D = Dl + 6 * pi + (rp * (rp + 1)) / 2;
              D[rp] += so;
              if (rp >= 1) D[rp - 1] += s1;
              if (rp >= 2) D[0] += s2;
            }
          }
        }
        {
          const int cA = min(32 * pr + lc, a0), cB = min(32 * pr + 16 + lc, a0);
#pragma unroll
          for (int mt = 0; mt < NT; ++mt) {
            double yJ0[4], yJ1[4];
            ld4(Yt + (size_t)mt * ytile + (size_t)cA * IYS + 4 * lr, yJ0);
            ld4(Yt + (size_t)mt * ytile + (size_t)cB * IYS + 4 * lr, yJ1);
#pragma unroll
            for (int ks = 0; ks < 4; ++ks)
              if (mt < NT - 1 || ks < nksl) {
                acc0 = __builtin_amdgcn_mfma_f64_16x16x4f64(ua[mt][ks], yJ0[ks], acc0, 0, 0, 0);
                acc1 = __builtin_amdgcn_mfma_f64_16x16x4f64(ua[mt][ks], yJ1[ks], acc1, 0, 0, 0);
              }
          }
        }
#pragma unroll
        for (int r = 0; r < 4; ++r) {
          const int q = rowq(I, lr + 4 * r);
          if (q >= 0) {
            double *rw = rowp(q) + 32 * pr + lc;
            rw[0] = acc0[r];
            rw[16] = acc1[r];
          }
        }
      };
      int e = 0;
      loads(0, aA0, aA1);
      for (; e + 1 < nun; e += 2) {
        loads(e + 1, aB0, aB1);
        unit(e, aA0, aA1);
        loads(min(e + 2, nun - 1), aA0, aA1);
        unit(e + 1, aB0, aB1);
      }
      if (e < nun) unit(e, aA0, aA1);
    }
    __syncthreads();
    if (b0 == 0) DRLGX_PROF(S, 38);
    else DRLGX_PROF(S, 47);
  };
  bool streamed = false;
  if constexpr (!kLds && kSNT > 0) {
    streamed = x.snt > 0 && (n_re > (x.wide ? 16 : 8) || (size_t)n1 * a0 * 8 > (size_t)(kStreamKB << 10));
  }
  if (streamed) {
    if constexpr (!kLds && kSNT > 0) {
      for (int b0 = 0; b0 < n_re;) {
        const int left = n_re - b0, nt = min(x.snt, (left + 7) >> 3), nb = min(8 * nt, left);
        if (nt >= 4) sbatch(b0, nb, std::integral_constant<int, kSNT >= 4 ? 4 : 1>{});
        else if (nt == 3) sbatch(b0, nb, std::integral_constant<int, 3>{});
        else if (nt == 2) sbatch(b0, nb, std::integral_constant<int, 2>{});
        else sbatch(b0, nb, std::integral_constant<int, 1>{});
        b0 += nb;
      }
    }
  } else {
    for (int b0 = 0; b0 < n_re;) {
      const int left = n_re - b0;
      if (left > 8 && x.wide) {
        const int nb = min(16, left);
        batch(b0, nb, std::true_type{});
        b0 += nb;
      } else {
        const int nb = min(8, left);
        batch(b0, nb, std::false_type{});
        b0 += nb;
      }
    }
  }
  DRLGX_PROF(S, 3);
  if (nn > 0) {
    if (tid < nn) {
      const double *rc = recs + (size_t)REC * fnew[tid];
      const double det = rc[6] * rc[9] - rc[7] * rc[8], id = 1.0 / det;
      const double i00 = rc[9] * id, i01 = -rc[7] * id, i10 = -rc[8] * id, i11 = rc[6] * id;
      double *g = gs + 12 * tid;
      for (int c = 0; c < 3; ++c) {
        g[c] = -(i00 * rc[c] + i01 * rc[3 + c]);
        g[3 + c] = -(i10 * rc[c] + i11 * rc[3 + c]);
      }
      g[6] = -(i00 * rc[10] + i01 * rc[11]);
      g[7] = -(i10 * rc[10] + i11 * rc[11]);
      g[8] = i00 * Rb * i00 + i01 * Rr * i01;
      g[9] = i00 * Rb * i10 + i01 * Rr * i11;
      g[10] = i10 * Rb * i10 + i11 * Rr * i11;
    }
    __syncthreads();
    for (int e = tid; e < 2 * nn * a0; e += kThreads) {
      const int rr = e / a0, c = e - rr * a0;
      const double *g = gs + 12 * (rr >> 1) + 3 * (rr & 1);
      rowp(n1 + rr)[c] = g[0] * rowp(3 * pn)[c] + g[1] * rowp(3 * pn + 1)[c] + g[2] * rowp(3 * pn + 2)[c];
    }
    if (tid < 2 * nn) {
      const double *g = gs + 12 * (tid >> 1);
      dl[n1 + tid] = g[3 * (tid & 1)] * dl[3 * pn] + g[3 * (tid & 1) + 1] * dl[3 * pn + 1] + g[3 * (tid & 1) + 2] * dl[3 * pn + 2] + g[6 + (tid & 1)];
    }
    __syncthreads();
    for (int e = tid; e < n * 2 * nn; e += kThreads) {
      const int q = e / (2 * nn), cc = e - q * 2 * nn;
      const double *g = gs + 12 * (cc >> 1);
      const double *r = rowp(q);
      double v = r[0] * g[3 * (cc & 1)] + r[1] * g[3 * (cc & 1) + 1] + r[2] * g[3 * (cc & 1) + 2];
      if (q >= n1 && ((q - n1) >> 1) == (cc >> 1)) {
        const int er = (q - n1) & 1, ec = cc & 1;
        v += er == ec ? (er ? g[10] : g[8]) : g[9];
      }
      rowp(q)[a0 + cc] = v;
    }
    __syncthreads();
  }
  DRLGX_PROF(S, 4);
  double *est_pose = S.est_pose + (size_t)inst * S.P_max * 4;
  double *pose_info = S.pose_info + (size_t)inst * S.P_max * 6;
  double *pose_tr = S.pose_tr + (size_t)inst * S.P_max;
  for (int i = tid; i < P; i += kThreads) {
    const Pose t{thp[4 * i], thp[4 * i + 1], thp[4 * i + 2], thp[4 * i + 3]};
    const double d0 = dl[3 * i], d1 = dl[3 * i + 1], d2 = dl[3 * i + 2];
    const Pose e = compose(t, make_pose(d0, d1, d2));
    est_pose[4 * i] = e.x; est_pose[4 * i + 1] = e.y; est_pose[4 * i + 2] = e.c; est_pose[4 * i + 3] = e.s;
    d_pose[3 * i] = d0; d_pose[3 * i + 1] = d1; d_pose[3 * i + 2] = d2;
    double c00, c10, c11, c20, c21, c22;
    if (i == pn) {
      const double *r0 = rowp(3 * pn), *r1 = rowp(3 * pn + 1), *r2 = rowp(3 * pn + 2);
      c00 = r0[0]; c10 = 0.5 * (r1[0] + r0[1]); c11 = r1[1]; c20 = 0.5 * (r2[0] + r0[2]); c21 = 0.5 * (r2[1] + r1[2]); c22 = r2[2];
    } else {
      const double *D = Dl + 6 * i;
      c00 = D[0]; c10 = D[1]; c11 = D[2]; c20 = D[3]; c21 = D[4]; c22 = D[5];
    }
    double *go = jd + 6 * i;
    go[0] = c00; go[1] = c10; go[2] = c11; go[3] = c20; go[4] = c21; go[5] = c22;
    pose_tr[i] = c00 + c11 + c22;
    double info[6];
    inv3_sym_fast(c00, c10, c20, c11, c21, c22, info);
    for (int k = 0; k < 6; ++k) pose_info[6 * i + k] = info[k];
    if (hand) {
      hand[4 * i] = e.x; hand[4 * i + 1] = e.y; hand[4 * i + 2] = e.c; hand[4 * i + 3] = e.s;
      for (int k = 0; k < 6; ++k) hand[4 * hand_cap + 6 * i + k] = info[k];
    }
  }
  {
    double *est_lm = S.est_lm + (size_t)inst * S.L_max * 2;
    double *lm_info = S.lm_info + (size_t)inst * S.L_max * 3;
    double *lm_tr = S.lm_tr + (size_t)inst * S.L_max;
    for (int j = kThreads - 1 - tid; j < L; j += kThreads) {
      const double dx = dl[3 * P + 2 * j], dy = dl[3 * P + 2 * j + 1];
      d_lm[2 * j] = dx; d_lm[2 * j + 1] = dy;
      const double ex = thl[2 * j] + dx, ey = thl[2 * j + 1] + dy;
      est_lm[2 * j] = ex;
      est_lm[2 * j + 1] = ey;
      if (hand) {
        thl[2 * j] = ex;
        thl[2 * j + 1] = ey;
      }
      const double *r0 = rowp(3 * P + 2 * j), *r1 = rowp(3 * P + 2 * j + 1);
      const double c00 = r0[3 + 2 * j], c11 = r1[3 + 2 * j + 1], cs = 0.5 * (r0[3 + 2 * j + 1] + r1[3 + 2 * j]);
      lm_tr[j] = c00 + c11;
      const double id = 1.0 / (c00 * c11 - cs * cs);
      lm_info[3 * j] = c11 * id;
      lm_info[3 * j + 1] = -cs * id;
      lm_info[3 * j + 2] = c00 * id;
    }
  }
  DRLGX_PROF(S, 5);
  if constexpr (kLds) {
    const int npair = (a + 1) >> 1;
    const int cp0 = tid & 31, r0 = tid >> 5;
    for (int cp = cp0; cp < npair; cp += 32)
      for (int q = r0; q < n; q += 16) reinterpret_cast<double2 *>(growp(q))[cp] = reinterpret_cast<const double2 *>(rowp(q))[cp];
  }
  if (tid == 0) {
    meta[0] = 1; meta[1] = P; meta[2] = L; meta[3] = M;
    cnt[C_ISAM] = cnt[C_ISAM] + 1;
    cnt[C_NEWP] = P;
    cnt[C_NEWL] = L;
    if (ictl[1]) atomicMin(S.status, DRLGX_E_NUMERIC);
    if (S.inc_stats) atomicAdd(S.inc_stats, 1ull);
  }
  DRLGX_PROF(S, 7);
  return true;
}

__device__ __forceinline__ void panel_invalidate(const DrlgxState &S, int inst, int tid) {
  if (S.jc && tid == 0) {
    inc_meta(S, inst)[0] = 0;
    if (S.inc_stats) atomicAdd(S.inc_stats + 1, 1ull);
  }
}

#pragma clang fp contract(fast)

template <int kSNT>
__device__ __forceinline__ bool inc_stage(const DrlgxState &S, const LaunchSel &sel, int lds_bytes, size_t smem_off) {
  const int tid = drlgx_tid(), bi = drlgx_bid();
  if (!S.jc || !sel.on(bi)) return false;
  const int inst = sel.base + bi;
  const int *cnt = S.cnt + (size_t)inst * DRLGX_CNT_STRIDE;
  if (cnt[C_FLAG]) return false;
  const int P = cnt[C_P], L = cnt[C_L], M = cnt[C_M];
  extern __shared__ __attribute__((aligned(16))) unsigned char smem_raw[];
  if (!inc_precheck(S, inst, P, tid, reinterpret_cast<int *>(smem_raw + smem_off))) return false;
  IncCtx x;
  bool lds_panel = false;
  if (!inc_plan(S, inst, P, lds_bytes, smem_off, x, lds_panel, sel.cap(S.P_max))) return false;
  const SimBox nobox{nullptr, nullptr, nullptr};
  bool done;
  if (lds_panel) {
    inc_pre<true, false>(S, x, tid, nullptr, SubBarrier{nullptr, 0, 0});
    __syncthreads();
    done = inc_post<true, kSNT>(S, x, L, M, nobox, tid);
  } else {
    inc_pre<false, false>(S, x, tid, nullptr, SubBarrier{nullptr, 0, 0});
    __syncthreads();
    done = inc_post<false, kSNT>(S, x, L, M, nobox, tid);
  }
  if (!done) __syncthreads();
  return done;
}
#pragma clang fp contract(off)
}
```

### drl_graph_exploration_amd/csrc/k_misc.hip

```cpp
#include "drlgx_dev.h"
#include "drlgx_fields.h"

namespace {

constexpr int kCopySplit = 8;
__device__ __forceinline__ void copy_panel_part(const DrlgxState &S, int s, int d, int part) {
  const int *ms = S.jc_meta + (size_t)s * 4;
  int *md = S.jc_meta + (size_t)d * 4;
  const int valid = ms[0], P = ms[1], L = ms[2], M = ms[3];
  if (threadIdx.x == 0 && part == 0) {
    md[0] = valid; md[1] = P; md[2] = L; md[3] = M;
  }
  if (valid != 1) return;
  const double *ps = S.jc + (size_t)s * S.jc_stride;
  double *pd = S.jc + (size_t)d * S.jc_stride;
  const int npair = (3 + 2 * L + 1) >> 1, rows = 3 * P + 2 * L;
  const int cp0 = threadIdx.x & 31, r0 = (threadIdx.x >> 5) + 8 * part, rs = 8 * kCopySplit;
  auto roff = [&](int q) -> size_t { return (size_t)(q < 3 * P ? q : q - 3 * P + 3 * S.P_max) * S.jc_ld; };
  for (int cp = cp0; cp < npair; cp += 32)
    for (int q = r0; q < rows; q += 4 * rs) {
      const int q1 = q + rs, q2 = q + 2 * rs, q3 = q + 3 * rs;
      const size_t o0 = roff(q), o1 = roff(min(q1, rows - 1)), o2 = roff(min(q2, rows - 1)), o3 = roff(min(q3, rows - 1));
      const double2 v0 = reinterpret_cast<const double2 *>(ps + o0)[cp], v1 = reinterpret_cast<const double2 *>(ps + o1)[cp];
      const double2 v2 = reinterpret_cast<const double2 *>(ps + o2)[cp], v3 = reinterpret_cast<const double2 *>(ps + o3)[cp];
      reinterpret_cast<double2 *>(pd + o0)[cp] = v0;
      if (q1 < rows) reinterpret_cast<double2 *>(pd + o1)[cp] = v1;
      if (q2 < rows) reinterpret_cast<double2 *>(pd + o2)[cp] = v2;
      if (q3 < rows) reinterpret_cast<double2 *>(pd + o3)[cp] = v3;
    }
  if (part == 0)
    for (int e = threadIdx.x; e < 6 * P; e += 256) S.jd[(size_t)d * S.P_max * 6 + e] = S.jd[(size_t)s * S.P_max * 6 + e];
}

__global__ __launch_bounds__(256) void k_copy_instances(const DrlgxField *fields, int n_fields, const int32_t *src,
                                                        const int32_t *dst, int src_off, int dst_off, int skip_mask, int only_cls,
                                                        const int *cnt, DrlgxState S, int panel) {
  const int i = blockIdx.y;
  const int f = blockIdx.x;
  const int s = (src ? src[i] : i) + src_off, d = (dst ? dst[i] : i) + dst_off;
  if (f >= n_fields) {
    if (panel) copy_panel_part(S, s, d, f - n_fields);
    return;
  }
  if ((fields[f].cls & skip_mask) || (only_cls >= 0 && fields[f].cls != only_cls)) return;
  const size_t stride = fields[f].stride;
  const char *sb = fields[f].base + (size_t)s * stride;
  char *db = fields[f].base + (size_t)d * stride;
  size_t live = fields[f].pad > 0 ? (size_t)fields[f].pad : stride;
  if (fields[f].unit && cnt) {
    const int *c = cnt + (size_t)s * DRLGX_CNT_STRIDE;
    const int k = fields[f].unit == 1 ? c[C_P] : fields[f].unit == 2 ? c[C_L] : c[C_M];
    const size_t b = ((size_t)(k > 0 ? k : 0) * (size_t)fields[f].unit_bytes + 15) & ~(size_t)15;
    live = b < stride ? b : stride;
  }
  if ((stride & 15) == 0) {
    const uint4 *sp = reinterpret_cast<const uint4 *>(sb);
    uint4 *dp = reinterpret_cast<uint4 *>(db);
    const size_t nq = live / 16;
    size_t k = threadIdx.x;
    for (; k + 256 < nq; k += 512) {
      const uint4 v0 = sp[k], v1 = sp[k + 256];
      dp[k] = v0; dp[k + 256] = v1;
    }
    if (k < nq) dp[k] = sp[k];
  } else {
    const uint32_t *sp = reinterpret_cast<const uint32_t *>(sb);
    uint32_t *dp = reinterpret_cast<uint32_t *>(db);
    const size_t nw = (live < stride ? live : stride) / 4;
    for (size_t k = threadIdx.x; k < nw; k += 256) dp[k] = sp[k];
  }
}

__global__ __launch_bounds__(256) void k_fetch_pack(const int *status, const int *cnt, int n_envs, int head, const unsigned char *src,
                                                    size_t bytes, unsigned char *out) {
  const size_t t = (size_t)blockIdx.x * 256 + threadIdx.x, nt = (size_t)gridDim.x * 256;
  int *h = reinterpret_cast<int *>(out);
  for (size_t i = t; i < (size_t)n_envs + 1; i += nt) h[i] = i == 0 ? status[0] : cnt[(i - 1) * DRLGX_CNT_STRIDE + C_P];
  unsigned char *o = out + head;
  if (((reinterpret_cast<uintptr_t>(src) | bytes) & 15) == 0) {
    const uint4 *s4 = reinterpret_cast<const uint4 *>(src);
    uint4 *o4 = reinterpret_cast<uint4 *>(o);
    for (size_t i = t; i < bytes / 16; i += nt) o4[i] = s4[i];
  } else {
    for (size_t i = t; i < bytes; i += nt) o[i] = src[i];
  }
}

__global__ __launch_bounds__(64) void k_rebase(DrlgxState S, int base0, int n) {
  const int inst = base0 + blockIdx.x;
  int *cnt = S.cnt + (size_t)inst * DRLGX_CNT_STRIDE;
  const int P = cnt[C_P], L = cnt[C_L];
  for (int i = threadIdx.x; i < P; i += 64) {
    for (int k = 0; k < 4; ++k)
      S.th_pose[((size_t)inst * S.P_max + i) * 4 + k] = S.est_pose[((size_t)inst * S.P_max + i) * 4 + k];
    for (int k = 0; k < 3; ++k) S.d_pose[((size_t)inst * S.P_max + i) * 3 + k] = 0.0;
  }
  for (int j = threadIdx.x; j < L; j += 64) {
    for (int k = 0; k < 2; ++k) {
      S.th_lm[((size_t)inst * S.L_max + j) * 2 + k] = S.est_lm[((size_t)inst * S.L_max + j) * 2 + k];
      S.d_lm[((size_t)inst * S.L_max + j) * 2 + k] = 0.0;
    }
  }
  if (threadIdx.x == 0) {
    cnt[C_ISAM] = 0;
    cnt[C_NEWP] = 0;
    cnt[C_NEWL] = 0;
    cnt[C_FLAG] = 0;
    if (S.jc_meta) S.jc_meta[(size_t)inst * 4] = 0;
  }
}

__global__ __launch_bounds__(64) void k_fix_rollouts(DrlgxState S, const int32_t *cand_env, int roll0) {
  const int c = blockIdx.x;
  const int env = cand_env[c], inst = roll0 + c;
  const int P = S.cnt[(size_t)inst * DRLGX_CNT_STRIDE + C_P];
  for (int e = threadIdx.x; e < P * 4; e += 64)
    S.est_pose[(size_t)inst * S.P_max * 4 + e] = S.est_pose[(size_t)env * S.P_max * 4 + e];
  if (threadIdx.x == 0) {
    S.parent[inst] = env;
    S.red[(size_t)inst * DRLGX_RED_STRIDE + R_DIST] = 0.0;
  }
}

__device__ __forceinline__ double utility_of(const DrlgxState &S, int inst, double dist) {
// ... 219 lines not shown
  return v > bv || (v == bv && i < bi);
}

__global__ __launch_bounds__(64) void k_greedy_plans(const float *score, int n_score, const int32_t *seg_begin, const int32_t *n_frontier,
                                                     const uint8_t *active, const double *actions_pad, const int32_t *n_act_pad,
                                                     int max_frontier, int max_actions, int32_t *choice, double *actions_out,
                                                     int32_t *n_actions_out) {
  const int e = blockIdx.x, lane = threadIdx.x;
  const int b = seg_begin[e];
  const int n = (active && !active[e]) || b < 0 ? 0 : min(min(n_frontier[e], max_frontier), n_score - b);
  const float *q = score + b;
  float bv = 0.f;
  int bi = -1;
  for (int i = lane; i < n; i += 64) {
    const float v = q[i];
    if (pick_beats(v, i, bv, bi)) { bv = v; bi = i; }
  }
  for (int o = 32; o > 0; o >>= 1) {
    const float ov = __shfl_xor(bv, o);
    const int oi = __shfl_xor(bi, o);
    if (pick_beats(ov, oi, bv, bi)) { bv = ov; bi = oi; }
  }
  int na = 0;
  const double *src = actions_pad;
  if (bi >= 0) {
    const size_t slot = (size_t)e * max_frontier + bi;
    na = min(max(n_act_pad[slot], 0), max_actions);
    src += slot * max_actions * 3;
  }
  double *dst = actions_out + (size_t)e * max_actions * 3;
  for (int k = lane; k < 3 * max_actions; k += 64) dst[k] = k < 3 * na ? src[k] : 0.0;
  if (lane == 0) {
    choice[e] = bi;
    n_actions_out[e] = na;
  }
}

__global__ __launch_bounds__(256) void k_cov_array(DrlgxState S, double *length, double *angle) {
  const int e = blockIdx.y, v = blockIdx.x * 256 + threadIdx.x;
  if (v >= S.V) return;
  const double *inf = S.vm_info + (size_t)e * 3 * S.V;
  double a, b, d;
  inv2_llt_s(inf[v], inf[S.V + v], inf[2 * S.V + v], a, b, d);
  const double half = 0.5 * (a - d), r = sqrt(half * half + b * b);
  const double lmax = 0.5 * (a + d) + r;
  double vx, vy;
  if (a >= d) {
    vx = half + r; vy = b;
    if (vx == 0.0 && vy == 0.0) { vx = 1.0; vy = 0.0; }
  } else {
    vx = b; vy = r - half;
  }
  length[(size_t)e * S.V + v] = fmin(sqrt(lmax), S.cfg.sigma0);
  angle[(size_t)e * S.V + v] = atan2(vy, vx);
}

}

void drlgx_launch_metrics(const DrlgxState &S, hipStream_t st, double sigma0, double *out) {
  hipLaunchKernelGGL(k_metrics, dim3(S.n_envs), dim3(256), 0, st, S, sigma0, out);
}
void drlgx_launch_plan_record(const DrlgxState &S, hipStream_t st, double sigma0, int a, int32_t *n_actions, double done_explored,
                              int max_steps, double *trace, int32_t *done) {
  hipLaunchKernelGGL(k_plan_record, dim3(S.n_envs), dim3(256), 0, st, S, sigma0, a, n_actions, done_explored, max_steps, trace, done);
}
void drlgx_launch_follow_select(const DrlgxState &S, hipStream_t st, const double *plan, const int32_t *n_actions, const int32_t *result,
                                const uint8_t *active, int steps, const double *fallback, double *act, int32_t *n_exec, int32_t *stop) {
  hipLaunchKernelGGL(k_follow_select, dim3(S.n_envs), dim3(64), 0, st, S, plan, n_actions, result, active, steps, fallback[0], fallback[1],
                     fallback[2], act, n_exec, stop);
}
void drlgx_launch_follow_record(const DrlgxState &S, hipStream_t st, double sigma0, int a, const double *act, int32_t *n_exec, int obstacles,
                                double done_explored, int max_steps, double *trace, int32_t *done, int32_t *stop) {
  hipLaunchKernelGGL(k_follow_record, dim3(S.n_envs), dim3(256), 0, st, S, sigma0, a, act, n_exec, obstacles, done_explored, max_steps, trace,
                     done, stop);
}
void drlgx_launch_obstacle_flags(const DrlgxState &S, hipStream_t st, uint8_t *out) {
  hipLaunchKernelGGL(k_obstacle_flags, dim3((S.n_envs + 127) / 128), dim3(128), 0, st, S, out);
}
void drlgx_launch_cov_array(const DrlgxState &S, hipStream_t st, double *length, double *angle) {
  hipLaunchKernelGGL(k_cov_array, dim3((S.V + 255) / 256, S.n_envs), dim3(256), 0, st, S, length, angle);
}
void drlgx_launch_copy(const DrlgxField *fields_dev, int n_fields, hipStream_t st, int n, const int32_t *src,
                       const int32_t *dst, int src_off, int dst_off, int skip_mask, const int *cnt, const DrlgxState *panel,
                       int only_cls) {
  if (n <= 0) return;
  const bool with_panel = panel && panel->jc;
  const dim3 cgrid(n_fields + (with_panel ? kCopySplit : 0), n);
  hipLaunchKernelGGL(k_copy_instances, cgrid, dim3(256), 0, st, fields_dev, n_fields, src, dst,
                     src_off, dst_off, skip_mask, only_cls, cnt, with_panel ? *panel : DrlgxState{}, with_panel ? 1 : 0);
}
void drlgx_launch_fetch_pack(const DrlgxState &S, hipStream_t st, const void *src, size_t bytes, void *out) {
  const size_t head = drlgx_fetch_head_bytes(S.n_envs);
  const int blocks = (int)std::min<size_t>(256, (head + bytes + 4095) / 4096);
  hipLaunchKernelGGL(k_fetch_pack, dim3(std::max(blocks, 1)), dim3(256), 0, st, S.status, S.cnt, S.n_envs, (int)head,
                     reinterpret_cast<const unsigned char *>(src), bytes, reinterpret_cast<unsigned char *>(out));
}
void drlgx_launch_rebase(const DrlgxState &S, hipStream_t st, int base0, int n) {
  hipLaunchKernelGGL(k_rebase, dim3(n), dim3(64), 0, st, S, base0, n);
}
void drlgx_launch_fix_rollouts(const DrlgxState &S, hipStream_t st, int n_cand, const int32_t *cand_env, int roll0) {
  hipLaunchKernelGGL(k_fix_rollouts, dim3(n_cand), dim3(64), 0, st, S, cand_env, roll0);
}
void drlgx_launch_rewards(const DrlgxState &S, hipStream_t st, int n_cand, const int32_t *cand_env, int roll0,
                          double *rewards) {
  hipLaunchKernelGGL(k_rewards, dim3((n_cand + 127) / 128), dim3(128), 0, st, S, n_cand, cand_env, roll0, rewards);
}
void drlgx_launch_utility(const DrlgxState &S, hipStream_t st, const double *dist, double *out, int mode) {
  hipLaunchKernelGGL(k_utility, dim3((S.n_envs + 127) / 128), dim3(128), 0, st, S, dist, out, mode);
}
void drlgx_launch_line_plan(const DrlgxState &S, hipStream_t st, int n_cand, const int32_t *cand_env, const double *goal,
                            double *actions, int32_t *n_actions) {
  hipLaunchKernelGGL(k_line_plan, dim3((n_cand + 127) / 128), dim3(128), 0, st, S, n_cand, cand_env, goal, actions,
                     n_actions);
}

int drlgx_greedy_plans(void *hip_stream, int n_envs, const float *score, int n_score, const int32_t *seg_begin, const int32_t *n_frontier,
                       const uint8_t *active, const double *actions_pad, const int32_t *n_act_pad, int max_frontier, int max_actions,
                       int32_t *choice, double *actions_out, int32_t *n_actions_out) {
  if (n_envs <= 0 || !score || n_score < 0 || !seg_begin || !n_frontier || !actions_pad || !n_act_pad || max_frontier <= 0 || max_actions <= 0 ||
      !choice || !actions_out || !n_actions_out)
    return DRLGX_E_INVALID;
  hipStream_t st = reinterpret_cast<hipStream_t>(hip_stream);
  hipLaunchKernelGGL(k_greedy_plans, dim3(n_envs), dim3(64), 0, st, score, n_score, seg_begin, n_frontier, active, actions_pad, n_act_pad,
                     max_frontier, max_actions, choice, actions_out, n_actions_out);
  return hipGetLastError() == hipSuccess ? DRLGX_OK : DRLGX_E_HIP;
}
```

### drl_graph_exploration_amd/csrc/k_slam_arrow.hip

```cpp

#pragma once
#include "k_inc.hip"
#include "k_sweep_ws.hip"
#include "arrow_carve.h"
namespace kslam {
#pragma clang fp contract(fast)
__device__ __forceinline__ bool inv3s(const double *a, double *o) {
  const double c00 = a[3] * a[5] - a[4] * a[4], c01 = a[2] * a[4] - a[1] * a[5], c02 = a[1] * a[4] - a[2] * a[3];
  const double det = a[0] * c00 + a[1] * c01 + a[2] * c02;
  const double id = fast_rcp(det);
  o[0] = c00 * id;
  o[1] = c01 * id;
  o[2] = c02 * id;
  o[3] = (a[0] * a[5] - a[2] * a[2]) * id;
  o[4] = (a[1] * a[2] - a[0] * a[4]) * id;
  o[5] = (a[0] * a[3] - a[1] * a[1]) * id;
  return a[0] > 0 && c00 > 0 && det > 0;
}
__device__ __forceinline__ double sym3(const double *a, int r, int c) {
  constexpr int idx[9] = {0, 1, 2, 1, 3, 4, 2, 4, 5};
  return a[idx[r * 3 + c]];
}

struct MaskIter {
// ... 907 lines not shown
        }
      }
    }
    if (zprof) {
      S.prof[105] = zt_stage; S.prof[106] = zt_k; S.prof[107] = zt_epi; S.prof[108] = zt_sum;
    }
    __syncthreads();
    for (int e = tid; e < nrows * 3; e += kThreads) {
      const int row = e / 3, b3 = e - 3 * row;
      Sc()[e] = ScL[e];
      if (mk_panel) pan_pose[(size_t)row * S.jc_ld + b3] = X[(size_t)row * ldx + np + 1 + b3] - SqL[e];
    }
  }

  __device__ __forceinline__ void pose_outputs(const DrlgxState &S) const {
    double *est_pose = S.est_pose + (size_t)inst * S.P_max * 4;
    double *pose_info = S.pose_info + (size_t)inst * S.P_max * 6;
    double *pose_tr = S.pose_tr + (size_t)inst * S.P_max;
    for (int i = tid; i < P; i += kThreads) {
      const double dp0 = X[(size_t)(3 * i) * ldx + np] - dz()[3 * i], dp1 = X[(size_t)(3 * i + 1) * ldx + np] - dz()[3 * i + 1],
                   dp2 = X[(size_t)(3 * i + 2) * ldx + np] - dz()[3 * i + 2];
      d_pose[3 * i] = dp0; d_pose[3 * i + 1] = dp1; d_pose[3 * i + 2] = dp2;
      const Pose t{thp[4 * i], thp[4 * i + 1], thp[4 * i + 2], thp[4 * i + 3]};
      const Pose e = compose(t, make_pose(dp0, dp1, dp2));
      est_pose[4 * i] = e.x; est_pose[4 * i + 1] = e.y; est_pose[4 * i + 2] = e.c; est_pose[4 * i + 3] = e.s;
      if (!full) continue;
      const double *ti = Ti + 6 * i, *sc = Sc() + 9 * i;
      const double c00 = ti[0] - sc[0], c10 = ti[1] - 0.5 * (sc[1] + sc[3]), c20 = ti[2] - 0.5 * (sc[2] + sc[6]);
      const double c11 = ti[3] - sc[4], c21 = ti[4] - 0.5 * (sc[5] + sc[7]), c22 = ti[5] - sc[8];
      pose_tr[i] = c00 + c11 + c22;
      inv3_sym_fast(c00, c10, c20, c11, c21, c22, pose_info + 6 * i);
      if (mk_panel) {
        double *go = S.jd + ((size_t)inst * S.P_max + i) * 6;
        go[0] = c00; go[1] = c10; go[2] = c11; go[3] = c20; go[4] = c21; go[5] = c22;
      }
    }
  }

  __device__ __forceinline__ void panel_finish(const DrlgxState &S, double *pan_pose, bool pn_done) const {
    const int pn = P - 1, ldg = S.jc_ld;
    double *pan_lm = pan_pose + (size_t)3 * S.P_max * ldg;
    for (int e = tid; e < 3 * P * 3 && !pn_done; e += kThreads) {
      const int row = e / 3, b = e - 3 * row;
      const double *zr = pan_pose + (size_t)row * ldg + 3, *xp = X + (size_t)(3 * pn + b) * ldx;
      double v = X[(size_t)row * ldx + np + 1 + b];
      for (int c = 0; c < np; ++c) v -= zr[c] * xp[c];
      pan_pose[(size_t)row * ldg + b] = v;
    }
    DRLGX_PROF(S, 103);
    for (int e = tid; e < np * np; e += kThreads) {
      const int r = e / np, c = e - r * np;
      pan_lm[(size_t)r * ldg + 3 + c] = -A[AT(max(r, c), min(r, c))];
    }
    for (int e = tid; e < np * 3; e += kThreads) {
      const int r = e / 3, b = e - 3 * r;
      pan_lm[(size_t)r * ldg + b] = pan_pose[(size_t)(3 * pn + b) * ldg + 3 + r];
    }
    DRLGX_PROF(S, 104);
    if (tid == 0) {
      int *meta = inc_meta(S, inst);
      meta[0] = 1; meta[1] = P; meta[2] = L; meta[3] = M;
      if (S.inc_stats) atomicAdd(S.inc_stats + 1, 1ull);
    }
  }

  __device__ __forceinline__ void counters(const DrlgxState &S) const {
    if (tid == 0) {
      if (!refresh) {
        cnt[C_ISAM] = count;
        cnt[C_NEWP] = P;
        cnt[C_NEWL] = L;
      }
      if (bad[0]) atomicMin(S.status, DRLGX_E_NUMERIC);
    }
    if (!refresh && !mk_panel) panel_invalidate(S, inst, tid);
  }
};

template <int NTW>
__device__ __forceinline__ void arrow_body(const DrlgxState &S, const LaunchSel &sel, int lds_bytes) {
  extern __shared__ __attribute__((aligned(16))) unsigned char smem_raw[];
  const int tid = drlgx_tid();
  const int bi = drlgx_bid();
  if (!sel.on(bi)) return;
  if (S.prof && tid == 0 && bi < 448) S.prof[128 + 2 * bi] = wall_clock64();
  if (inc_stage<ISNT>(S, sel, lds_bytes, 0)) {
    if (S.prof && tid == 0 && bi < 448) S.prof[129 + 2 * bi] = wall_clock64();
    return;
  }
  const int inst = sel.base + bi;
  const bool want = sel.map_on(bi), full = want || S.jc != nullptr;
  const bool refresh = S.cnt[(size_t)inst * DRLGX_CNT_STRIDE + C_FLAG] != 0;
  if (refresh && !(sel.map_last_only && sel.n_act && want)) return;
  ArrowCtx c;
  if (!c.setup<NTW>(S, smem_raw, lds_bytes, inst, full, refresh)) {
    if (tid == 0) atomicMin(S.status, DRLGX_E_CAPACITY);
    return;
  }
  DRLGX_PROF(S, 0);
  c.relinearise();
  c.factor_tables(S);
  DRLGX_PROF(S, 1);
  c.blocks(S);
  DRLGX_PROF(S, 2);
  __syncthreads();
  c.leaves_factor();
  DRLGX_PROF(S, 3);
  c.leaves_rhs();
  __syncthreads();
  DRLGX_PROF(S, 4);
  c.separators_down();
  c.root();
  __syncthreads();
  c.separators_up();
  DRLGX_PROF(S, 5);
  c.leaves_up();
  __syncthreads();
  c.clear_system();
  __syncthreads();
  DRLGX_PROF(S, 10);
  c.landmark_system();
  __syncthreads();
  DRLGX_PROF(S, 6);
  c.sweep<NTW>(S);
  __syncthreads();
  DRLGX_PROF(S, 7);
  c.landmark_outputs(S);
  DRLGX_PROF(S, 8);
  double *pan_pose = c.mk_panel ? S.jc + (size_t)inst * S.jc_stride : nullptr;
  const bool pn_done = c.pose_products(S, pan_pose);
  __syncthreads();
  DRLGX_PROF(S, 101);
  c.pose_outputs(S);
  DRLGX_PROF(S, 9);
  if (c.mk_panel) {
    __syncthreads();
    DRLGX_PROF(S, 102);
    c.panel_finish(S, pan_pose, pn_done);
  }
  c.counters(S);
}

template <int NTW>
__global__ __launch_bounds__(kThreads) void k_slam_arrow(DRLGX_KS_PARAM, LaunchSel sel, int lds_bytes) {
  const DrlgxState &S = DRLGX_KS_REF;
  arrow_body<NTW>(S, sel, lds_bytes);
}
#pragma clang fp contract(off)
}
```

### drl_graph_exploration_amd/csrc/k_step.hip

```cpp
#include "drlgx_dev.h"

#include "k_sim.hip"
#include "k_sweep.hip"
#include "k_slam_common.hip"
#include "k_inc.hip"
#include "k_slam.hip"
#include "k_slam_arrow.hip"
#include "k_slam_host.hip"
#include "k_map.hip"
#include "k_em.hip"
#include "k_og.hip"

namespace kstep {

__host__ __device__ inline size_t sim_lds_bytes(int LG, int P_max) { return drlgx_sim_lds_bytes(LG, P_max); }

template <int FT>
__device__ __forceinline__ void step_once(const DrlgxState &S, const LaunchSel &sel, const double *odom, int odom_stride, int n_measure,
                                          int lds_bytes, int map_chunk) {
  static_assert(kslam::kThreads == kmap::kThreads, "the fused kernel runs both stages with one workgroup size");
  extern __shared__ __attribute__((aligned(16))) unsigned char step_smem[];
  const int tid = drlgx_tid();
  const int bi = drlgx_bid();
  if (S.prof && tid == 0 && bi < 448) S.prof[128 + 2 * bi] = wall_clock64();
  const int pc = sel.cap(S.P_max);
  const size_t sim_bytes = sim_lds_bytes(S.LG, pc);
  int *sub_cnt = reinterpret_cast<int *>(step_smem + sim_bytes - 16);
  double *sim_dyn = reinterpret_cast<double *>(step_smem + 2 * DRLGX_MT_STRIDE * sizeof(uint32_t));
  double *lmbox = reinterpret_cast<double *>(step_smem + sim_bytes - 16 - (size_t)2 * S.LG * 8);
  const kslam::SimBox box{(n_measure == 2 && !sel.simlog) ? sim_dyn : nullptr, reinterpret_cast<const int *>(sim_dyn + 2 * S.LG + 2), lmbox};
  kmap::LadderEntry lo{true, 0.0, -1, 0, 0};
  if (tid < S.lo_ntab) lo.pv = S.lo_pv[tid];
  kslam::SlamCtx ctx;
  bool pre = false, accepted = false, inc_try = false;
  double od3[3] = {0, 0, 0};
  int P0 = 0, L0 = 0, M0 = 0, isam = 0, pan_L0 = -1, pan_M0 = -1;
  ksim::SimPre spre;
  spre.have = tid < 64 && !sel.simlog && sel.on(bi);
  if (sel.on(bi)) {
    const int inst = sel.base + bi;
    const int *cnt = S.cnt + (size_t)inst * DRLGX_CNT_STRIDE;
    P0 = cnt[C_P]; L0 = cnt[C_L]; M0 = cnt[C_M]; isam = cnt[C_ISAM];
    int meta0 = 0, meta1 = 0;
    if (S.jc) {
      const int4 mv = *reinterpret_cast<const int4 *>(kslam::inc_meta(S, inst));
      meta0 = mv.x & 0x7fffffff;
      meta1 = mv.y;
      pan_L0 = mv.z;
      pan_M0 = mv.w;
    }
    const double *od = odom + (size_t)bi * odom_stride + (size_t)sel.act_idx * 3;
    od3[0] = od[0]; od3[1] = od[1]; od3[2] = od[2];
    if (spre.have) ksim::sim_preload(S, inst, tid, n_measure, spre);
    accepted = ksim::move_accepted(S, od3[0], od3[1], P0);
    inc_try = accepted && kslam::inc_precheck(S, inst, P0 + 1, tid, sub_cnt, meta0, meta1, isam);
    const int Lb = min(S.L_max, L0 + 48), Mb = min(S.M_max, M0 + 48);
    pre = accepted && !inc_try && (3 * (P0 + 1) + 1 + 15) / 16 <= kslam::kDenseTiles && kslam::SlamCtx::big_fits(sim_bytes, lds_bytes, P0 + 1, Lb, Mb);
    if (pre) ctx.setup<true>(S, step_smem, sim_bytes, lds_bytes, inst, P0 + 1, Lb, Mb);
  }
  if (tid == 0) {
    sub_cnt[0] = 0;
    sub_cnt[1] = -1;
  }
  __syncthreads();
  if (tid < 64) {
    uint32_t *l0 = reinterpret_cast<uint32_t *>(step_smem);
    uint32_t *l1 = l0 + DRLGX_MT_STRIDE;
    double *dyn = sim_dyn;
    if (sel.simlog)
      ksim::replay_step_body(S, sel, odom, odom_stride, tid, sub_cnt + 1);
    else
      ksim::sim_step_body(S, sel, odom, odom_stride, n_measure, l0, l1, dyn, tid, nullptr, nullptr, nullptr, true, sub_cnt + 1,
                          n_measure == 2 ? lmbox : nullptr, sel.on(bi) ? P0 : -1, L0, M0, spre);
  } else if (pre) {
    ctx.front<true>(S, tid, P0, L0, M0, P0, L0, isam + 1, false, od3, kslam::SubBarrier{sub_cnt, kslam::kThreads / 64 - 1, 0});
  } else if (inc_try) {
    kslam::IncCtx ix;
    bool inc_lds = false;
    if (kslam::inc_plan(S, sel.base + bi, P0 + 1, lds_bytes, sim_bytes, ix, inc_lds, pc, pan_L0, pan_M0)) {
      const kslam::SubBarrier sb{sub_cnt, kslam::kThreads / 64 - 1, 0};
      if (inc_lds) kslam::inc_pre<true, true>(S, ix, tid, od3, sb);
      else kslam::inc_pre<false, true>(S, ix, tid, od3, sb);
    }
  }
  __syncthreads();
  DRLGX_PROF(S, 32);
  if (accepted && tid >= 64 && !sel.simlog) {
    uint32_t *g = S.mt + (size_t)(sel.base + bi) * 2 * DRLGX_MT_STRIDE;
    const uint32_t *img = reinterpret_cast<const uint32_t *>(step_smem);
    for (int i = tid - 64; i < 2 * DRLGX_MT_STRIDE; i += kslam::kThreads - 64) g[i] = img[i];
  }
  const kmap::MapCarve map_carve(pc, map_chunk, S.V, false);
  const bool hand = map_carve.stage + 16 <= sim_bytes - 16;
  const double *lm_lds = nullptr;
  bool inc_done = false;
  if (inc_try) {
    kslam::IncCtx ix;
    bool inc_lds = false;
    if (kslam::inc_plan(S, sel.base + bi, P0 + 1, lds_bytes, sim_bytes, ix, inc_lds, pc, pan_L0, pan_M0)) {
      double *hp = hand ? reinterpret_cast<double *>(step_smem) : nullptr;
      inc_done = inc_lds ? kslam::inc_post<true, 0>(S, ix, sub_cnt[2], sub_cnt[3], box, tid, hp, pc)
                         : kslam::inc_post<false, 0>(S, ix, sub_cnt[2], sub_cnt[3], box, tid, hp, pc);
      if (inc_done) lm_lds = ix.thl;
      else __syncthreads();
    }
  }
  if (!inc_done)
    kslam::slam_finish<FT>(S, sel, lds_bytes, sim_bytes, ctx, pre, sub_cnt + 1, hand ? reinterpret_cast<double *>(step_smem) : nullptr, &lm_lds, box, pc);
  __syncthreads();
  const bool handed = hand && lm_lds != nullptr;
  if (sel.on(bi)) {
    const bool appended = sub_cnt[1] >= 0;
    lo.P = appended ? sub_cnt[1] : P0;
    lo.L = appended ? sub_cnt[2] : L0;
    lo.flag = appended ? 0 : 1;
  }
  const unsigned char *map_masks = step_smem + map_carve.mask;
  if (!handed || reinterpret_cast<const unsigned char *>(lm_lds + 2 * (size_t)S.L_max) > map_masks) lm_lds = nullptr;
  if (!sel.skip_map) kmap::map_body<false>(S, sel, 1, map_chunk, handed, lm_lds, lo);
  if (S.prof && tid == 0 && bi < 448) S.prof[129 + 2 * bi] = wall_clock64();
}

template <int FT>
__global__ __launch_bounds__(kslam::kThreads) void k_step(DrlgxState S, LaunchSel sel, const double *odom, int odom_stride,
                                                          int n_measure, int lds_bytes, int map_chunk) {
  step_once<FT>(S, sel, odom, odom_stride, n_measure, lds_bytes, map_chunk);
}

template <int FT>
__global__ __launch_bounds__(kslam::kThreads) void k_step_ref(DrlgxStateConst Sp, LaunchSel sel, const double *odom, int odom_stride,
                                                              int n_measure, int lds_bytes, int map_chunk) {
  if (__builtin_amdgcn_readfirstlane((int)threadIdx.x >> 6) == 0) drlgx_warm_state(Sp);
  step_once<FT>(*(const DrlgxState *)Sp, sel, odom, odom_stride, n_measure, lds_bytes, map_chunk);
}

template <int FT>
__global__ __launch_bounds__(kslam::kThreads) void k_step_loop(DRLGX_KS_PARAM, LaunchSel sel, const double *odom, int odom_stride,
                                                               int n_measure, int lds_bytes, int map_chunk, int a_end) {
  const DrlgxState &S = DRLGX_KS_REF;
  const int bi = blockIdx.x;
  const int n_mine = sel.n_act ? min(a_end, sel.n_act[bi]) : a_end;
  if (sel.active && !sel.active[bi]) return;
  for (int a = sel.act_idx; a < n_mine; ++a) {
    LaunchSel one = sel;
    one.act_idx = a;
    one.pcap = min(sel.pcap + (a - sel.act_idx), S.P_max);
    step_once<FT>(S, one, odom, odom_stride, n_measure, lds_bytes, map_chunk);
    __syncthreads();
  }
}

__device__ __forceinline__ void step_arrow_once(const DrlgxState &S, const LaunchSel &sel, const double *odom, int odom_stride, int n_measure,
                                                int lds_bytes, int map_chunk) {
  extern __shared__ __attribute__((aligned(16))) unsigned char step_smem[];
  const int tid = drlgx_tid();
  if (tid < 64) {
    uint32_t *l0 = reinterpret_cast<uint32_t *>(step_smem);
    uint32_t *l1 = l0 + DRLGX_MT_STRIDE;
    double *dyn = reinterpret_cast<double *>(step_smem + 2 * DRLGX_MT_STRIDE * sizeof(uint32_t));
    if (sel.simlog) ksim::replay_step_body(S, sel, odom, odom_stride, tid);
    else ksim::sim_step_body(S, sel, odom, odom_stride, n_measure, l0, l1, dyn, tid);
  }
  __syncthreads();
  kslam::arrow_body<0>(S, sel, lds_bytes);
  __syncthreads();
  if (!sel.skip_map) kmap::map_body<false>(S, sel, 1, map_chunk);
}
__global__ __launch_bounds__(kslam::kThreads) void k_step_arrow(DRLGX_KS_PARAM, LaunchSel sel, const double *odom, int odom_stride,
                                                                int n_measure, int lds_bytes, int map_chunk) {
  const DrlgxState &S = DRLGX_KS_REF;
  step_arrow_once(S, sel, odom, odom_stride, n_measure, lds_bytes, map_chunk);
}
__global__ __launch_bounds__(kslam::kThreads) void k_step_arrow_loop(DRLGX_KS_PARAM, LaunchSel sel, const double *odom, int odom_stride,
                                                                     int n_measure, int lds_bytes, int map_chunk, int a_end) {
  const DrlgxState &S = DRLGX_KS_REF;
  const int bi = blockIdx.x;
  const int n_mine = sel.n_act ? min(a_end, sel.n_act[bi]) : a_end;
  if (sel.active && !sel.active[bi]) return;
  for (int a = sel.act_idx; a < n_mine; ++a) {
    LaunchSel one = sel;
    one.act_idx = a;
    one.pcap = min(sel.pcap + (a - sel.act_idx), S.P_max);
    step_arrow_once(S, one, odom, odom_stride, n_measure, lds_bytes, map_chunk);
    __syncthreads();
  }
}

}
// ... 45 lines not shown
```

### drl_graph_exploration_amd/engine.py

```python
import ctypes as C
import math

import numpy as np
import torch

from . import _lib
from .config import DrlgxConfig, start_pose


def _p(t):
    return C.c_void_p(t.data_ptr()) if t is not None else None


_NP_OF = {torch.float32: np.float32, torch.float64: np.float64, torch.int32: np.int32, torch.int64: np.int64, torch.uint8: np.uint8,
          torch.bool: np.bool_, torch.int16: np.int16, torch.int8: np.int8}


class Engine(object):
    def __init__(self, cfg, n_envs, n_rollouts=0, device=0):
        if not isinstance(cfg, DrlgxConfig):
            raise TypeError("cfg must be a DrlgxConfig")
        if not torch.cuda.is_available():
            raise _lib.DrlgxError("no HIP device visible: the drlgx engine has no CPU fallback")
        self.L = _lib.lib()
# ... 372 lines not shown
    def cov_array(self):
        self.use_torch_stream()
        ln = torch.empty(self.n_envs, self.rows, self.cols, dtype=torch.float64, device=self.device)
        an = torch.empty_like(ln)
        self._chk(self.L.drlgx_cov_array(self.h, _p(ln), _p(an)))
        return ln, an

    def line_plan(self, cand_env, goals):
        self.use_torch_stream()
        n = cand_env.numel()
        A = self.cfg.max_actions
        actions = torch.zeros(n, A, 3, dtype=torch.float64, device=self.device)
        n_act = torch.zeros(n, dtype=torch.int32, device=self.device)
        self._chk(self.L.drlgx_line_plan(self.h, n, _p(cand_env), _p(goals), _p(actions), _p(n_act)))
        return actions, n_act

    def lookahead(self, cand_env, actions, n_actions, max_n_actions=None):
        self.use_torch_stream()
        n = cand_env.numel()
        rewards = torch.empty(n, dtype=torch.float64, device=self.device)
        if max_n_actions is None:
            self._chk(self.L.drlgx_lookahead(self.h, n, _p(cand_env), _p(actions), _p(n_actions), _p(rewards)))
        else:
            self._chk(self.L.drlgx_lookahead_bounded(self.h, n, _p(cand_env), _p(actions), _p(n_actions), int(max_n_actions),
                                                     _p(rewards)))
        return rewards

    def graph_capacity(self):
        if not hasattr(self, "_gcap"):
            a, b, c = C.c_int32(), C.c_int32(), C.c_int32()
            self._chk(self.L.drlgx_graph_capacity(self.h, C.byref(a), C.byref(b), C.byref(c)))
            self._gcap = (a.value, b.value, c.value)
        return self._gcap

    def graph(self, plan=False):
        self.use_torch_stream()
        if not hasattr(self, "_gcap"):
            a, b, c = C.c_int32(), C.c_int32(), C.c_int32()
            self._chk(self.L.drlgx_graph_capacity(self.h, C.byref(a), C.byref(b), C.byref(c)))
            self._gcap = (a.value, b.value, c.value)
        mn, me, mf = self._gcap
        dev = self.device
        node_off = torch.empty(self.n_envs + 1, dtype=torch.int32, device=dev)
        edge_off = torch.empty(self.n_envs + 1, dtype=torch.int32, device=dev)
        x = torch.empty(mn, 5, dtype=torch.float32, device=dev)
        ei = torch.empty(2 * me, dtype=torch.int64, device=dev)
        ea = torch.empty(me, dtype=torch.float32, device=dev)
        nfr = torch.empty(self.n_envs, dtype=torch.int32, device=dev)
        fxy = torch.zeros(self.n_envs, mf, 2, dtype=torch.float64, device=dev)
        near = torch.empty(self.n_envs, dtype=torch.int32, device=dev)
        self._chk(self.L.drlgx_graph(self.h, _p(node_off), _p(edge_off), _p(x), _p(ei), _p(ea), _p(nfr), _p(fxy), _p(near)))
        extra = {}
        if plan:
            if getattr(self, "_pad_env", None) is None:
                self._pad_env = torch.arange(self.n_envs, device=dev, dtype=torch.int32).repeat_interleave(mf).contiguous()
            acts, n_act = self.line_plan(self._pad_env, fxy.view(-1, 2))
            extra = dict(actions_pad=acts.view(self.n_envs, mf, -1, 3), n_act_pad=n_act.view(self.n_envs, mf))
        if plan:
            node_off_h, edge_off_h, nfr_h, n_act_h = self.fetch(node_off, edge_off, nfr, extra["n_act_pad"])
            extra["n_act_pad_h"] = n_act_h
        else:
            node_off_h, edge_off_h, nfr_h = self.fetch(node_off, edge_off, nfr)
        N, E = int(node_off_h[-1]), int(edge_off_h[-1])
        counts = (node_off[1:] - node_off[:-1]).to(torch.int64)
        batch = torch.repeat_interleave(torch.arange(self.n_envs, device=dev), counts, output_size=N)
        return dict(x=x[:N], edge_index=ei[:2 * E].view(2, E), edge_attr=ea[:E], node_off=node_off, edge_off=edge_off,
                    batch=batch, n_frontier=nfr, frontier_xy=fxy, nearest_frontier_node=near,
                    max_graph_edges=int(np.diff(edge_off_h).max()) if self.n_envs else 0,
                    node_off_h=node_off_h, edge_off_h=edge_off_h, n_frontier_h=nfr_h, **extra)

    def snapshot(self, slot=0):
        self.use_torch_stream()
        self._chk(self.L.drlgx_snapshot(self.h, slot))

    def restore(self, slot=0):
        self.use_torch_stream()
        self._chk(self.L.drlgx_restore(self.h, slot))

    def inc_stats(self, reset=False):
        out = (C.c_int64 * 2)()
        self._chk(self.L.drlgx_inc_stats_host(self.h, out, 1 if reset else 0))
        return int(out[0]), int(out[1])

    def timing_enable(self, on=True):
        self._chk(self.L.drlgx_timing_enable(self.h, int(on)))

    def timing_read(self):
        ms = (C.c_double * _lib.N_TIMERS)()
        n = (C.c_int64 * _lib.N_TIMERS)()
        self._chk(self.L.drlgx_timing_read_host(self.h, ms, n))
        names = ["sim", "slam", "map", "copy", "graph", "step", "t6", "t7"]
        return {names[i]: (ms[i], n[i]) for i in range(_lib.N_TIMERS)}

    def counts(self, inst):
        out = (C.c_int32 * 5)()
        self._chk(self.L.drlgx_get_counts_host(self.h, inst, out))
        return dict(poses=out[0], landmarks=out[1], factors=out[2], step=out[3], isam_count=out[4])

    def counts_dev(self):
        self.use_torch_stream()
        out = torch.empty(self.n_envs, 5, dtype=torch.int32, device=self.device)
        self._chk(self.L.drlgx_counts(self.h, _p(out)))
        return out

    def poses(self, inst):
        P = self.counts(inst)["poses"]
        xyt = np.zeros((P, 3))
        info = np.zeros((P, 3, 3))
        dp = C.POINTER(C.c_double)
        self._chk(self.L.drlgx_get_poses_host(self.h, inst, xyt.ctypes.data_as(dp), info.ctypes.data_as(dp)))
        return xyt, info

    def landmarks(self, inst):
        n = self.counts(inst)["landmarks"]
        keys = np.zeros(n, dtype=np.int32)
        xy = np.zeros((n, 2))
        info = np.zeros((n, 2, 2))
        dp = C.POINTER(C.c_double)
        self._chk(self.L.drlgx_get_landmarks_host(self.h, inst, keys.ctypes.data_as(C.POINTER(C.c_int32)),
                                                  xy.ctypes.data_as(dp), info.ctypes.data_as(dp)))
        return keys, xy, info

    def cov_traces(self, inst):
        c = self.counts(inst)
        lm = np.zeros(c["landmarks"])
        ps = np.zeros(c["poses"])
        dp = C.POINTER(C.c_double)
        self._chk(self.L.drlgx_get_cov_traces_host(self.h, inst, lm.ctypes.data_as(dp), ps.ctypes.data_as(dp)))
        return lm, ps

    def virtual_map(self, inst):
        V = self.rows * self.cols
        prob = np.zeros(V)
        info = np.zeros((V, 2, 2))
        tr = np.zeros(V)
        upd = np.zeros(V, dtype=np.uint8)
        dp = C.POINTER(C.c_double)
        self._chk(self.L.drlgx_get_virtual_map_host(self.h, inst, prob.ctypes.data_as(dp), info.ctypes.data_as(dp),
                                                    tr.ctypes.data_as(dp), upd.ctypes.data_as(C.POINTER(C.c_uint8))))
        return prob.reshape(self.rows, self.cols), info, tr.reshape(self.rows, self.cols), upd

    def ground_truth(self, inst):
        veh = np.zeros(3)
        lms = np.zeros((max(self.cfg.num_landmarks, 1), 2))
        dp = C.POINTER(C.c_double)
        self._chk(self.L.drlgx_get_ground_truth_host(self.h, inst, veh.ctypes.data_as(dp), lms.ctypes.data_as(dp)))
        return veh, lms[:self.cfg.num_landmarks]

    def adjacency(self, inst):
        c = self.counts(inst)
        N = c["poses"] + c["landmarks"]
        A = np.zeros((N, N))
        X = np.zeros(N)
        dp = C.POINTER(C.c_double)
        self._chk(self.L.drlgx_get_adjacency_host(self.h, inst, A.ctypes.data_as(dp), X.ctypes.data_as(dp)))
        return A, X

    def factors(self, inst):
        m = self.counts(inst)["factors"]
        pose = np.zeros(m, dtype=np.int32)
        key = np.zeros(m, dtype=np.int32)
        b = np.zeros(m)
        r = np.zeros(m)
        dp, ip = C.POINTER(C.c_double), C.POINTER(C.c_int32)
        self._chk(self.L.drlgx_get_factors_host(self.h, inst, pose.ctypes.data_as(ip), key.ctypes.data_as(ip),
                                                b.ctypes.data_as(dp), r.ctypes.data_as(dp)))
# ... 7 lines not shown
```

### include/drlgx.h

```cpp
#ifndef DRLGX_H
#define DRLGX_H

#include <stddef.h>
#include <stdint.h>

#ifdef __cplusplus
extern "C" {
#endif

#define DRLGX_OK 0
#define DRLGX_E_INVALID (-1)
#define DRLGX_E_NODEVICE (-2)
#define DRLGX_E_CAPACITY (-3)
#define DRLGX_E_HIP (-4)
#define DRLGX_E_NUMERIC (-5)

#define DRLGX_ALG_EM_AOPT 0
#define DRLGX_ALG_EM_DOPT 1

typedef struct drlgx_config {
  double bearing_noise, range_noise, min_bearing, max_bearing, min_range, max_range;
  double translation_noise, rotation_noise;
  double env_min_x, env_max_x, env_min_y, env_max_y, safe_distance;
  double map_min_x, map_max_x, map_min_y, map_max_y;
// ... 60 lines not shown
                  int algorithm, double *uncertainty_out_dev, double *cost_out_dev, double *info_out_dev);
int drlgx_em_cost_steps(drlgx_engine *e, int n_cand, const int32_t *cand_env_dev, const double *actions_dev, const int32_t *n_actions_dev,
                        const uint8_t *core_dev, const double *distance_dev, int algorithm, double *uncertainty_out_dev,
                        double *cost_out_dev, double *info_out_dev);

int drlgx_og_cost(drlgx_engine *e, int n_cand, const int32_t *cand_env_dev, const double *actions_dev, const int32_t *n_actions_dev,
                  double *entropy_out_dev, double *cost_out_dev, double *prob_out_dev);

int drlgx_set_sampler_parameter(drlgx_engine *e, double max_nodes, double safe_distance, int dubins_control_model_enabled);
int drlgx_set_sampler_obstacles(drlgx_engine *e, int enabled);
int drlgx_set_dubins_library_host(drlgx_engine *e, const double *params);
int drlgx_dubins_library(drlgx_engine *e, int capacity, int32_t *n_out, double *end_xytheta, double *v, double *w, int32_t *num_steps);
int drlgx_set_dubins_prefilter(drlgx_engine *e, int enabled);
int drlgx_set_dubins_leaf_scoring(drlgx_engine *e, int enabled);
int drlgx_em_plan_leaves(drlgx_engine *e, int capacity, int32_t *n_out_host, int32_t *has_steps_out_host, int32_t *cand_env_out_dev,
                         double *actions_out_dev, int32_t *n_actions_out_dev, uint8_t *core_out_dev, double *distance_out_dev,
                         double *cost_out_dev);
int drlgx_em_plan(drlgx_engine *e, int n_sel, const int32_t *env_sel_dev, const int32_t *halton_start_dev, int max_tree_nodes,
                  int algorithm, double *plan_out_dev, int32_t *n_actions_out_dev, double *cost_out_dev, int32_t *result_out_dev,
                  int32_t *n_leaves_out_dev, int32_t *halton_next_out_dev, double *nodes_out_dev, int32_t *n_nodes_out_dev);
int drlgx_rrt_plan(drlgx_engine *e, int n_sel, const int32_t *env_sel_dev, const int32_t *goal_key_dev, const double *goal_xy_dev,
                   const int32_t *halton_start_dev, int max_tree_nodes, double *plan_out_dev, int32_t *n_actions_out_dev,
                   int32_t *result_out_dev, int32_t *halton_next_out_dev, double *nodes_out_dev, int32_t *n_nodes_out_dev);

int drlgx_set_fixed_landmarks_host(drlgx_engine *e, int n_fixed, const double *xy);
int drlgx_set_planner_parameter(drlgx_engine *e, double angle_weight, double distance_weight0, double distance_weight1,
                                double occupancy_threshold, double max_edge_length, int algorithm);

int drlgx_utility(drlgx_engine *e, const double *dist_dev, double *out_dev);
int drlgx_uncertainty_em(drlgx_engine *e, int algorithm, double *out_dev);
int drlgx_explored(drlgx_engine *e, double *out_dev);

int drlgx_metrics(drlgx_engine *e, double sigma0, double *out_dev);
int drlgx_cov_array(drlgx_engine *e, double *length_dev, double *angle_dev);


int drlgx_line_plan(drlgx_engine *e, int n_cand, const int32_t *cand_env_dev, const double *goal_dev,
                    double *actions_dev, int32_t *n_actions_dev);

int drlgx_lookahead(drlgx_engine *e, int n_cand, const int32_t *cand_env_dev, const double *actions_dev,
                    const int32_t *n_actions_dev, double *rewards_dev);

int drlgx_lookahead_bounded(drlgx_engine *e, int n_cand, const int32_t *cand_env_dev, const double *actions_dev,
                            const int32_t *n_actions_dev, int max_n_actions, double *rewards_dev);


int drlgx_graph_capacity(const drlgx_engine *e, int *max_nodes, int *max_edges, int *max_frontier);
int drlgx_graph(drlgx_engine *e, int32_t *node_off_dev, int32_t *edge_off_dev, float *x_dev,
                int64_t *edge_index_dev, float *edge_attr_dev, int32_t *n_frontier_dev, double *frontier_xy_dev,
                int32_t *nearest_frontier_node_dev);


int drlgx_get_counts_host(drlgx_engine *e, int inst, int32_t out[5]);
int drlgx_counts(drlgx_engine *e, int32_t *counts_dev);
int drlgx_get_poses_host(drlgx_engine *e, int inst, double *xytheta, double *information);
int drlgx_get_landmarks_host(drlgx_engine *e, int inst, int32_t *keys, double *xy, double *information);
int drlgx_get_cov_traces_host(drlgx_engine *e, int inst, double *lm_trace, double *pose_trace);
int drlgx_vm_shape(const drlgx_engine *e, int *rows, int *cols);
int drlgx_get_virtual_map_host(drlgx_engine *e, int inst, double *prob, double *info, double *cov_trace,
                               uint8_t *updated);
int drlgx_get_ground_truth_host(drlgx_engine *e, int inst, double *vehicle_xytheta, double *landmarks_xy);
int drlgx_get_adjacency_host(drlgx_engine *e, int inst, double *adjacency, double *features);
int drlgx_get_factors_host(drlgx_engine *e, int inst, int32_t *pose, int32_t *key, double *bearing, double *range);
int drlgx_get_landmark_order_host(const drlgx_engine *e, int32_t *order);

int drlgx_snapshot(drlgx_engine *e, int slot);
int drlgx_restore(drlgx_engine *e, int slot);

#define DRLGX_N_TIMERS 8
int drlgx_timing_enable(drlgx_engine *e, int on);
int drlgx_timing_read_host(drlgx_engine *e, double ms[DRLGX_N_TIMERS], int64_t launches[DRLGX_N_TIMERS]);

int drlgx_debug_phase_clocks_host(drlgx_engine *e, int arm, int64_t *out );

int drlgx_debug_gemm_tile_rows(int m, int n, int k_slices, int transpose_a);

int drlgx_debug_map_form(int form);

int drlgx_debug_map_compact_ok(const drlgx_engine *e, int p_bound);

int drlgx_debug_disc_cells_bound(double radius_cells);

int drlgx_inc_stats_host(drlgx_engine *e, int64_t out[2], int reset);


size_t drlgx_gcn_workspace_bytes(int n_nodes, int n_edges, int hidden, int out_dim);
int drlgx_gcn_forward(void *hip_stream, int n_nodes, int n_edges, int in_dim, int hidden, int out_dim,
                      const float *x, const int64_t *edge_index, const float *edge_attr, const float *W1,
                      const float *b1, const float *W2, const float *b2, const float *Wf, const float *bf,
                      const float *dropout_mask , float *out ,
                      void *ws_dev);
int drlgx_gcn_forward_batched(void *hip_stream, int n_nodes, int n_edges, int in_dim, int hidden, int out_dim,
                              const float *x, const int64_t *edge_index, const float *edge_attr, const float *W1,
                              const float *b1, const float *W2, const float *b2, const float *Wf, const float *bf,
                              const float *dropout_mask, float *out, void *ws_dev, int n_graphs,
                              const int32_t *node_off, const int32_t *edge_off, int max_edges_per_graph);
int drlgx_gcn_backward(void *hip_stream, int n_nodes, int n_edges, int in_dim, int hidden, int out_dim,
                       const float *x, const int64_t *edge_index, const float *edge_attr, const float *W1,
                       const float *W2, const float *Wf, const float *dropout_mask, const float *d_out,
                       float *dW1, float *db1, float *dW2, float *db2, float *dWf, float *dbf, void *ws_dev);


size_t drlgx_ggnn_workspace_bytes(int n_nodes, int n_edges, int hidden, int n_layers, int out_dim);
int drlgx_ggnn_forward(void *hip_stream, int n_nodes, int n_edges, int in_dim, int hidden, int n_layers, int out_dim,
                       const float *x, const int64_t *edge_index, const float *edge_attr,
                       const float *weight , const float *w_ih , const float *w_hh,
                       const float *b_ih, const float *b_hh, const float *Wf, const float *bf,
                       const float *dropout_mask , float *out, void *ws_dev,
                       int n_graphs, const int32_t *node_off, const int32_t *edge_off, int max_edges_per_graph);
int drlgx_ggnn_backward(void *hip_stream, int n_nodes, int n_edges, int in_dim, int hidden, int n_layers, int out_dim,
                        const float *x, const int64_t *edge_index, const float *edge_attr, const float *weight,
                        const float *w_ih, const float *w_hh, const float *Wf, const float *dropout_mask, const float *d_out,
                        float *d_weight, float *d_w_ih, float *d_w_hh, float *d_b_ih, float *d_b_hh,
                        float *dWf, float *dbf, void *ws_dev);


size_t drlgx_unet_workspace_bytes(int n_nodes, int n_edges, int n_graphs, int max_graph_nodes, int hidden, int depth, double pool_ratio,
                                  int out_dim);
int drlgx_unet_forward(void *hip_stream, int n_nodes, int n_edges, int in_dim, int hidden, int depth, double pool_ratio, int out_dim,
                       const float *x, const int64_t *edge_index, const float *edge_attr, const float *const *params,
                       const float *dropout_mask , float *out, void *ws_dev, size_t ws_bytes,
                       int n_graphs, const int32_t *node_off, const int32_t *edge_off, int max_graph_nodes);
int drlgx_unet_backward(void *hip_stream, int n_nodes, int n_edges, int in_dim, int hidden, int depth, double pool_ratio, int out_dim,
                        const float *x, const int64_t *edge_index, const float *edge_attr, const float *const *params,
                        const float *dropout_mask, const float *d_out, float *const *grads, void *ws_dev, size_t ws_bytes,
                        int n_graphs, int max_graph_nodes);
int drlgx_unet_kept_nodes(void *hip_stream, int n_nodes, int n_edges, int hidden, int depth, double pool_ratio, int out_dim, void *ws_dev,
                          size_t ws_bytes, int n_graphs, int max_graph_nodes, int level, int32_t *perm_out, int *count_host);
int drlgx_unet_topk(void *hip_stream, int n_nodes, int n_graphs, const int32_t *node_off, const float *scores, double pool_ratio,
                    int32_t *pooled_node_off, int32_t *pooled_edge_off, int32_t *perm, int32_t *inverse);
int drlgx_unet_augment_filter(void *hip_stream, int n_nodes, int n_edges, const int64_t *edge_index, const float *edge_attr, int n_graphs,
                              const int32_t *node_off, const int32_t *edge_off, int max_graph_nodes, const int32_t *perm,
                              const int32_t *pooled_node_off, const int32_t *pooled_edge_off, int64_t pooled_capacity,
                              int64_t *pooled_edge_index, float *pooled_edge_attr, int32_t *pooled_edge_count);


int drlgx_replay_collate(void *hip_stream, int n_graphs, const int64_t *desc_dev, const float *pool_x, int in_dim,
                         const int64_t *pool_ei, int64_t pool_edges, const float *pool_ea, float *x_out, int64_t *ei_out,
                         int64_t n_edges_total, float *ea_out, int64_t *batch_out,
                         int32_t *node_off_out , int32_t *edge_off_out ,
                         const float *pool_q , float *q_out );
int drlgx_replay_collate_pair(void *hip_stream, int n_graphs, const int64_t *desc_dev, const float *pool_x, int in_dim,
                              const int64_t *pool_ei, int64_t pool_edges, const float *pool_ea, float *x_out, int64_t *ei_out,
                              int64_t n_edges_total, float *ea_out, int64_t *batch_out, int32_t *node_off_out, int32_t *edge_off_out,
                              const int64_t *desc2_dev, const float *pool_q, float *q2_out);
int drlgx_dqn_targets(void *hip_stream, int n_samples, const float *q1, const int64_t *meta_dev, const double *r_dev,
                      double gamma, int64_t n_nodes_total, double *a_batch, double *y_batch);
int drlgx_dqn_loss_grad(void *hip_stream, int n_nodes, const float *pred, const double *action, const double *y,
                        double batch, double *loss_out, float *d_pred);
int drlgx_adam_step(void *hip_stream, int n_tensors, float *const *params, const float *const *grads,
                    float *const *exp_avg, float *const *exp_avg_sq, const int64_t *sizes, double lr, double beta1,
                    double beta2, double eps, int64_t step, double grad_clamp);
int drlgx_adam_step_scaled(void *hip_stream, int n_tensors, float *const *params, const float *const *grads,
                    float *const *exp_avg, float *const *exp_avg_sq, const int64_t *sizes, double lr, double beta1,
                    double beta2, double eps, int64_t step, double grad_clamp, double grad_scale);

typedef struct drlgx_csr_cache {
  float *deg, *selfw, *ax;
  int32_t *ptr_dst, *end_dst, *ptr_src, *end_src;
  int32_t *nbr_dst, *nbr_src;
  float *wn_dst, *wn_src;
} drlgx_csr_cache;
int drlgx_replay_cache_csr(void *hip_stream, int n_graphs, const int32_t *node_off, const int32_t *edge_off, int max_edges_per_graph,
                           const float *x, int in_dim, const int64_t *edge_index, int64_t edge_row_stride, const float *edge_attr,
                           const drlgx_csr_cache *cache);
int drlgx_gcn_collate_csr(void *hip_stream, int n_graphs, const int64_t *desc_dev, const drlgx_csr_cache *cache, int n_nodes,
// ... 41 lines not shown
```

Baseline: 4.049 million env-steps/sec.

## Defer snapshot panel copy on lazy restore and read from source panel

On a lazy restore the Jacobian/covariance panel is no longer copied from the snapshot slot. The metadata is flagged as living in the source slot. The incremental SLAM pre/post stages read unchanged columns straight from the snapshot panel and write only the updated rows to the instance panel. Any path that needs the full panel first settles it with an in-kernel copy. This is meant to cut the bulk panel copy traffic per restore, at the cost of extra branching, a flag bit in the metadata, and correctness risk across several kernels. A debug panel readback API is also added.

Result: faster. 4.192 million env-steps/sec (median of 6 runs) (+3.6%).

```diff
diff --git a/drl_graph_exploration_amd/_lib.py b/drl_graph_exploration_amd/_lib.py
--- a/drl_graph_exploration_amd/_lib.py
+++ b/drl_graph_exploration_amd/_lib.py
@@ -34,7 +34,7 @@
     "drlgx_get_poses_host", "drlgx_get_landmarks_host", "drlgx_get_cov_traces_host", "drlgx_vm_shape",
     "drlgx_get_virtual_map_host", "drlgx_get_ground_truth_host", "drlgx_get_adjacency_host", "drlgx_get_factors_host",
     "drlgx_get_landmark_order_host", "drlgx_snapshot", "drlgx_restore", "drlgx_timing_enable",
-    "drlgx_timing_read_host", "drlgx_debug_phase_clocks_host", "drlgx_debug_gemm_tile_rows", "drlgx_debug_map_form", "drlgx_debug_map_compact_ok", "drlgx_debug_disc_cells_bound", "drlgx_inc_stats_host", "drlgx_gcn_workspace_bytes", "drlgx_gcn_forward", "drlgx_gcn_forward_batched", "drlgx_gcn_backward",
+    "drlgx_timing_read_host", "drlgx_debug_phase_clocks_host", "drlgx_debug_gemm_tile_rows", "drlgx_debug_map_form", "drlgx_debug_map_compact_ok", "drlgx_debug_disc_cells_bound", "drlgx_inc_stats_host", "drlgx_debug_panel_host", "drlgx_gcn_workspace_bytes", "drlgx_gcn_forward", "drlgx_gcn_forward_batched", "drlgx_gcn_backward",
     "drlgx_replay_collate", "drlgx_replay_collate_pair", "drlgx_dqn_targets", "drlgx_dqn_loss_grad", "drlgx_dqn_arena_bytes", "drlgx_dqn_arena_views", "drlgx_dqn_prepare", "drlgx_dqn_forward_backward", "drlgx_replay_cache_csr", "drlgx_gcn_collate_csr", "drlgx_gcn_forward_prebuilt", "drlgx_adam_step", "drlgx_adam_step_scaled", "drlgx_normalise_rewards",
     "drlgx_segment_softmax", "drlgx_segment_softmax_backward", "drlgx_mean_pool", "drlgx_mean_pool_backward",
     "drlgx_ggnn_workspace_bytes", "drlgx_ggnn_forward", "drlgx_ggnn_backward",
@@ -131,6 +131,8 @@
     L.drlgx_debug_map_compact_ok.argtypes = [vp, C.c_int]
     L.drlgx_debug_disc_cells_bound.argtypes = [C.c_double]
     L.drlgx_inc_stats_host.argtypes = [vp, C.POINTER(C.c_int64), C.c_int]
+    if os.environ.get("DRLGX_LIB_DEV") is None or hasattr(L, "drlgx_debug_panel_host"):
+        L.drlgx_debug_panel_host.argtypes = [vp, C.c_int, ip, dp, C.c_size_t]
     L.drlgx_gcn_workspace_bytes.restype = C.c_size_t
     L.drlgx_gcn_workspace_bytes.argtypes = [C.c_int, C.c_int, C.c_int, C.c_int]
     L.drlgx_gcn_forward.argtypes = [vp] + [C.c_int] * 5 + [vp] * 12
diff --git a/drl_graph_exploration_amd/csrc/drlgx_dev.h b/drl_graph_exploration_amd/csrc/drlgx_dev.h
--- a/drl_graph_exploration_amd/csrc/drlgx_dev.h
+++ b/drl_graph_exploration_amd/csrc/drlgx_dev.h
@@ -119,6 +119,29 @@
   return t;
 }
 
+constexpr int kPanelInSrc = (int)0x80000000u;
+
+template <int kNT>
+__device__ __forceinline__ void drlgx_copy_panel_body(const double *jc, size_t jc_stride, int jc_ld, int P_max, int s, int d, int P, int L,
+                                                      int part, int nparts, int tid) {
+  const double *ps = jc + (size_t)s * jc_stride;
+  double *pd = const_cast<double *>(jc) + (size_t)d * jc_stride;
+  const int npair = (3 + 2 * L + 1) >> 1, rows = 3 * P + 2 * L;
+  const int cp0 = tid & 31, r0 = (tid >> 5) + (kNT / 32) * part, rs = (kNT / 32) * nparts;
+  auto roff = [&](int q) -> size_t { return (size_t)(q < 3 * P ? q : q - 3 * P + 3 * P_max) * jc_ld; };
+  for (int cp = cp0; cp < npair; cp += 32)
+    for (int q = r0; q < rows; q += 4 * rs) {
+      const int q1 = q + rs, q2 = q + 2 * rs, q3 = q + 3 * rs;
+      const size_t o0 = roff(q), o1 = roff(min(q1, rows - 1)), o2 = roff(min(q2, rows - 1)), o3 = roff(min(q3, rows - 1));
+      const double2 v0 = reinterpret_cast<const double2 *>(ps + o0)[cp], v1 = reinterpret_cast<const double2 *>(ps + o1)[cp];
+      const double2 v2 = reinterpret_cast<const double2 *>(ps + o2)[cp], v3 = reinterpret_cast<const double2 *>(ps + o3)[cp];
+      reinterpret_cast<double2 *>(pd + o0)[cp] = v0;
+      if (q1 < rows) reinterpret_cast<double2 *>(pd + o1)[cp] = v1;
+      if (q2 < rows) reinterpret_cast<double2 *>(pd + o2)[cp] = v2;
+      if (q3 < rows) reinterpret_cast<double2 *>(pd + o3)[cp] = v3;
+    }
+}
+
 struct LaunchSel {
   int base;
   int n;
@@ -580,7 +603,8 @@
                        const int32_t *dst, int src_off, int dst_off, int skip_mask,
                        const int *cnt = nullptr,
                        const DrlgxState *panel = nullptr,
-                       int only_cls = -1);
+                       int only_cls = -1,
+                       int panel_mode = 1);
 void drlgx_launch_rebase(const DrlgxState &S, hipStream_t st, int base0, int n);
 inline size_t drlgx_fetch_head_bytes(int n_envs) { return ((size_t)(n_envs + 1) * sizeof(int) + 15) & ~(size_t)15; }
 void drlgx_launch_fetch_pack(const DrlgxState &S, hipStream_t st, const void *src, size_t bytes, void *out);
diff --git a/drl_graph_exploration_amd/csrc/drlgx_engine.cpp b/drl_graph_exploration_amd/csrc/drlgx_engine.cpp
--- a/drl_graph_exploration_amd/csrc/drlgx_engine.cpp
+++ b/drl_graph_exploration_amd/csrc/drlgx_engine.cpp
@@ -576,7 +576,7 @@
 static void settle(drlgx_engine *e) {
   if (e->owed_slot < 0) return;
   drlgx_launch_copy(e->fields_dev, (int)e->fields.size(), e->stream, e->S.n_envs, nullptr, nullptr, snapshot_base(e, e->owed_slot), 0, 0,
-                    nullptr, nullptr, 1);
+                    nullptr, &e->S, 1, 3);
   e->owed_slot = -1;
 }
 
@@ -1741,7 +1741,7 @@
   const DrlgxState &S = e->S;
   ScopedTimer t(e, 3);
   drlgx_launch_copy(e->fields_dev, (int)e->fields.size(), e->stream, S.n_envs, nullptr, nullptr, snapshot_base(e, slot), 0,
-                    e->restore_eager ? 0 : 1, e->S.cnt, &S);
+                    e->restore_eager ? 0 : 1, e->S.cnt, &S, -1, e->restore_eager ? 1 : 2);
   e->owed_slot = e->restore_eager ? -1 : slot;
   e->pbound = e->snap_pbound[slot];
   return check_launch(e);
@@ -1780,6 +1780,29 @@
   return DRLGX_OK;
 }
 
+int drlgx_debug_panel_host(drlgx_engine *e, int inst, int32_t meta[4], double *panel, size_t panel_cap) {
+  DRLGX_ENTER(e);
+  if (!INST_OK(e, inst) || !meta) return DRLGX_E_INVALID;
+  const DrlgxState &S = e->S;
+  meta[0] = meta[1] = meta[2] = meta[3] = 0;
+  if (!S.jc) return DRLGX_OK;
+  int r = fetch(e, meta, S.jc_meta + (size_t)inst * 4, 4 * sizeof(int32_t));
+  if (r) return r;
+  HIPCHK(e, hipStreamSynchronize(e->stream));
+  if (!panel || meta[0] != 1) return DRLGX_OK;
+  const int P = meta[1], L = meta[2];
+  if (P < 0 || P > S.P_max || L < 0 || L > S.L_max) return DRLGX_E_INVALID;
+  const size_t cols = 3 + 2 * (size_t)L, rows = 3 * (size_t)P + 2 * (size_t)L;
+  if (rows * cols > panel_cap) return DRLGX_E_INVALID;
+  const double *src = S.jc + (size_t)inst * S.jc_stride;
+  if (P > 0) HIPCHK(e, hipMemcpy2DAsync(panel, cols * 8, src, (size_t)S.jc_ld * 8, cols * 8, 3 * (size_t)P, hipMemcpyDeviceToHost, e->stream));
+  if (L > 0)
+    HIPCHK(e, hipMemcpy2DAsync(panel + 3 * (size_t)P * cols, cols * 8, src + 3 * (size_t)S.P_max * S.jc_ld, (size_t)S.jc_ld * 8, cols * 8,
+                               2 * (size_t)L, hipMemcpyDeviceToHost, e->stream));
+  HIPCHK(e, hipStreamSynchronize(e->stream));
+  return DRLGX_OK;
+}
+
 int drlgx_timing_enable(drlgx_engine *e, int on) {
   DRLGX_ENTER_OWING(e);
   if (!e) return DRLGX_E_INVALID;
diff --git a/drl_graph_exploration_amd/csrc/k_inc.hip b/drl_graph_exploration_amd/csrc/k_inc.hip
--- a/drl_graph_exploration_amd/csrc/k_inc.hip
+++ b/drl_graph_exploration_amd/csrc/k_inc.hip
@@ -128,7 +128,8 @@
 }
 
 template <bool kLds, bool kSub>
-__device__ __forceinline__ void inc_pre(const DrlgxState &S, const IncCtx &x, int tid, const double *odom3, SubBarrier sb) {
+__device__ __forceinline__ void inc_pre(const DrlgxState &S, const IncCtx &x, int tid, const double *odom3, SubBarrier sb,
+                                        const double *src_panel = nullptr) {
   const int ft = kSub ? tid - 64 : tid, fn = kSub ? kThreads - 64 : kThreads, lane = tid & 63;
   auto bar = [&]() {
     if constexpr (kSub) sb.sync(lane);
@@ -136,7 +137,9 @@
   };
   const int inst = x.inst, P = x.P, pn = x.pn, pp = x.pp, L0 = x.L0, n1 = x.n1, a0 = x.a0;
   double *gpan = S.jc + (size_t)inst * S.jc_stride;
+  const double *span = src_panel ? src_panel : gpan;
   auto growp = [&](int q) -> double * { return gpan + (size_t)(q < 3 * P ? q : q + 3 * (S.P_max - P)) * S.jc_ld; };
+  auto srowp = [&](int q) -> const double * { return span + (size_t)(q < 3 * P ? q : q + 3 * (S.P_max - P)) * S.jc_ld; };
   auto rowp = [&](int q) -> double * {
     if constexpr (kLds) return x.cwl + (size_t)q * x.ldw;
     else return gpan + (size_t)(q < 3 * P ? q : q + 3 * (S.P_max - P)) * S.jc_ld;
@@ -182,7 +185,7 @@
     for (int cp = cp0; cp < npair; cp += 32)
       for (int qq = r0; qq < nr; qq += 4 * rs) {
         const int q0 = qq, q1 = qq + rs, q2 = qq + 2 * rs, q3 = qq + 3 * rs;
-        auto src = [&](int q) { const int c = min(q, nr - 1); return reinterpret_cast<const double2 *>(growp(c < 3 * pn ? c : c + 3))[cp]; };
+        auto src = [&](int q) { const int c = min(q, nr - 1); return reinterpret_cast<const double2 *>(srowp(c < 3 * pn ? c : c + 3))[cp]; };
         const double2 v0 = src(q0), v1 = src(q1), v2 = src(q2), v3 = src(q3);
         auto dst = [&](int q, const double2 &v) { if (q < nr) reinterpret_cast<double2 *>(rowp(q < 3 * pn ? q : q + 3))[cp] = v; };
         dst(q0, v0); dst(q1, v1); dst(q2, v2); dst(q3, v3);
@@ -200,7 +203,9 @@
     for (int qq = ft; qq < n1 - 3; qq += fn) {
       const int q = qq < 3 * pn ? qq : qq + 3;
       double *r = rowp(q);
-      const double t0 = r[0], t1 = r[1], t2 = r[2];
+      const double *rs = r;
+      if constexpr (!kLds) rs = srowp(q);
+      const double t0 = rs[0], t1 = rs[1], t2 = rs[2];
       r[0] = f00 * t0 + f01 * t1 + f02 * t2;
       r[1] = f10 * t0 + f11 * t1 + f12 * t2;
       r[2] = f20 * t0 + f21 * t1 + f22 * t2;
@@ -209,7 +214,11 @@
   bar();
   for (int e = ft; e < 3 * a0; e += fn) {
     const int r = e / a0, c = e - r * a0;
-    double v = fq[3 * r] * rowp(3 * pp)[c] + fq[3 * r + 1] * rowp(3 * pp + 1)[c] + fq[3 * r + 2] * rowp(3 * pp + 2)[c];
+    auto prev = [&](int k) -> double {
+      if constexpr (kLds) return rowp(3 * pp + k)[c];
+      else return (c < 3 ? rowp(3 * pp + k) : srowp(3 * pp + k))[c];
+    };
+    double v = fq[3 * r] * prev(0) + fq[3 * r + 1] * prev(1) + fq[3 * r + 2] * prev(2);
     if (c == r) v += 1.0 / (c < 2 ? S.w_trans : S.w_rot);
     rowp(3 * pn + r)[c] = v;
   }
@@ -219,7 +228,7 @@
 
 template <bool kLds, int kSNT = ISNT>
 __device__ __forceinline__ bool inc_post(const DrlgxState &S, const IncCtx &x, int L, int M, const SimBox &box, int tid,
-                                         double *hand = nullptr, int hand_cap = 0) {
+                                         double *hand = nullptr, int hand_cap = 0, const double *src_panel = nullptr) {
   const int lane = tid & 63, wave = tid >> 6, lc = lane & 15, lr = lane >> 4;
   const int inst = x.inst, P = x.P, pn = x.pn, L0 = x.L0, M0 = x.M0, n1 = x.n1, n1p = x.n1p, a0 = x.a0;
   int *meta = inc_meta(S, inst);
@@ -228,10 +237,15 @@
   int *fre = x.fre, *fnew = x.fnew, *fslot = x.fslot, *ictl = x.ictl;
   double *recs = x.recs, *gs = x.gs, *vvec = x.vvec, *wks = x.wks, *thp = x.thp, *thl = x.thl, *dl = x.dl, *Dl = x.Dl, *Y = x.Y;
   double *gpan = S.jc + (size_t)inst * S.jc_stride;
+  const double *span = (!kLds && src_panel) ? src_panel : gpan;
   auto growp = [&](int q) -> double * { return gpan + (size_t)(q < 3 * P ? q : q + 3 * (S.P_max - P)) * S.jc_ld; };
   auto rowp = [&](int q) -> double * {
     if constexpr (kLds) return x.cwl + (size_t)q * x.ldw;
     else return gpan + (size_t)(q < 3 * P ? q : q + 3 * (S.P_max - P)) * S.jc_ld;
+  };
+  auto srowp = [&](int q) -> const double * {
+    if constexpr (kLds) return x.cwl + (size_t)q * x.ldw;
+    else return ((q >= 3 * pn && q < 3 * P) ? gpan : span) + (size_t)(q < 3 * P ? q : q + 3 * (S.P_max - P)) * S.jc_ld;
   };
   int *cnt = S.cnt + (size_t)inst * DRLGX_CNT_STRIDE;
   double *d_pose = S.d_pose + (size_t)inst * S.P_max * 3;
@@ -292,8 +306,9 @@
         double c0[4], c1[4], c2[4], l0[4], l1[4];
 #pragma unroll
         for (int u = 0; u < 4; ++u) {
-          const double *r = rowp(min(q0 + u * RS, n1 - 1));
-          c0[u] = r[0]; c1[u] = r[1]; c2[u] = r[2]; l0[u] = r[cl]; l1[u] = r[cl + 1];
+          const int qc = min(q0 + u * RS, n1 - 1);
+          const double *r = rowp(qc), *rs = srowp(qc);
+          c0[u] = r[0]; c1[u] = r[1]; c2[u] = r[2]; l0[u] = rs[cl]; l1[u] = rs[cl + 1];
         }
 #pragma unroll
         for (int u = 0; u < 4; ++u) {
@@ -392,9 +407,10 @@
         const int it = e / npr, pr = e - it * npr, I = wave + kWaves * it;
 #pragma unroll
         for (int r = 0; r < 4; ++r) {
-          const double *rw = rowp(16 * I + lr + 4 * r) + 32 * pr + lc;
-          c0[r] = rw[0];
-          c1[r] = rw[16];
+          const int q = 16 * I + lr + 4 * r, c = 32 * pr + lc;
+          const double *rs = srowp(q);
+          c0[r] = (c < 3 ? rowp(q) : rs)[c];
+          c1[r] = rs[c + 16];
         }
       };
       auto unit = [&](int e, v4d &acc0, v4d &acc1) {
@@ -786,6 +802,17 @@
         batch(b0, nb, std::false_type{});
         b0 += nb;
       }
+      span = gpan;
+    }
+    if constexpr (!kLds) {
+      if (span != gpan) {
+        for (int qq = wave; qq < n1 - 3; qq += kWaves) {
+          const int q = qq < 3 * pn ? qq : qq + 3;
+          for (int c = 3 + lane; c < a0; c += 64) rowp(q)[c] = srowp(q)[c];
+        }
+        span = gpan;
+        __syncthreads();
+      }
     }
   }
   DRLGX_PROF(S, 3);
@@ -907,11 +934,24 @@
   }
 }
 
+__device__ __forceinline__ void inc_settle(const DrlgxState &S, const LaunchSel &sel) {
+  if (!S.jc || sel.vm_from < 0) return;
+  const int tid = drlgx_tid(), bi = drlgx_bid();
+  int *meta = inc_meta(S, sel.base + bi);
+  const int m0 = meta[0];
+  if (!(m0 & kPanelInSrc)) return;
+  drlgx_copy_panel_body<kThreads>(S.jc, S.jc_stride, S.jc_ld, S.P_max, sel.vm_from + bi, sel.base + bi, meta[1], meta[2], 0, 1, tid);
+  __syncthreads();
+  if (tid == 0) meta[0] = m0 & ~kPanelInSrc;
+  __syncthreads();
+}
+
 #pragma clang fp contract(fast)
 
 template <int kSNT>
 __device__ __forceinline__ bool inc_stage(const DrlgxState &S, const LaunchSel &sel, int lds_bytes, size_t smem_off) {
   const int tid = drlgx_tid(), bi = drlgx_bid();
+  inc_settle(S, sel);
   if (!S.jc || !sel.on(bi)) return false;
   const int inst = sel.base + bi;
   const int *cnt = S.cnt + (size_t)inst * DRLGX_CNT_STRIDE;
diff --git a/drl_graph_exploration_amd/csrc/k_misc.hip b/drl_graph_exploration_amd/csrc/k_misc.hip
--- a/drl_graph_exploration_amd/csrc/k_misc.hip
+++ b/drl_graph_exploration_amd/csrc/k_misc.hip
@@ -4,31 +4,20 @@
 namespace {
 
 constexpr int kCopySplit = 8;
-__device__ __forceinline__ void copy_panel_part(const DrlgxState &S, int s, int d, int part) {
+__device__ __forceinline__ void copy_panel_part(const DrlgxState &S, int s, int d, int part, int mode) {
   const int *ms = S.jc_meta + (size_t)s * 4;
   int *md = S.jc_meta + (size_t)d * 4;
-  const int valid = ms[0], P = ms[1], L = ms[2], M = ms[3];
+  const int valid = ms[0] & ~kPanelInSrc, P = ms[1], L = ms[2], M = ms[3];
   if (threadIdx.x == 0 && part == 0) {
-    md[0] = valid; md[1] = P; md[2] = L; md[3] = M;
+    if (mode != 3) {
+      md[0] = (mode == 2 && valid == 1) ? (valid | kPanelInSrc) : valid; md[1] = P; md[2] = L; md[3] = M;
+    } else if (valid == 1) {
+      md[0] = valid;
+    }
   }
   if (valid != 1) return;
-  const double *ps = S.jc + (size_t)s * S.jc_stride;
-  double *pd = S.jc + (size_t)d * S.jc_stride;
-  const int npair = (3 + 2 * L + 1) >> 1, rows = 3 * P + 2 * L;
-  const int cp0 = threadIdx.x & 31, r0 = (threadIdx.x >> 5) + 8 * part, rs = 8 * kCopySplit;
-  auto roff = [&](int q) -> size_t { return (size_t)(q < 3 * P ? q : q - 3 * P + 3 * S.P_max) * S.jc_ld; };
-  for (int cp = cp0; cp < npair; cp += 32)
-    for (int q = r0; q < rows; q += 4 * rs) {
-      const int q1 = q + rs, q2 = q + 2 * rs, q3 = q + 3 * rs;
-      const size_t o0 = roff(q), o1 = roff(min(q1, rows - 1)), o2 = roff(min(q2, rows - 1)), o3 = roff(min(q3, rows - 1));
-      const double2 v0 = reinterpret_cast<const double2 *>(ps + o0)[cp], v1 = reinterpret_cast<const double2 *>(ps + o1)[cp];
-      const double2 v2 = reinterpret_cast<const double2 *>(ps + o2)[cp], v3 = reinterpret_cast<const double2 *>(ps + o3)[cp];
-      reinterpret_cast<double2 *>(pd + o0)[cp] = v0;
-      if (q1 < rows) reinterpret_cast<double2 *>(pd + o1)[cp] = v1;
-      if (q2 < rows) reinterpret_cast<double2 *>(pd + o2)[cp] = v2;
-      if (q3 < rows) reinterpret_cast<double2 *>(pd + o3)[cp] = v3;
-    }
-  if (part == 0)
+  if (mode != 2) drlgx_copy_panel_body<256>(S.jc, S.jc_stride, S.jc_ld, S.P_max, s, d, P, L, part, kCopySplit, threadIdx.x);
+  if (part == 0 && mode != 3)
     for (int e = threadIdx.x; e < 6 * P; e += 256) S.jd[(size_t)d * S.P_max * 6 + e] = S.jd[(size_t)s * S.P_max * 6 + e];
 }
 
@@ -39,7 +28,7 @@
   const int f = blockIdx.x;
   const int s = (src ? src[i] : i) + src_off, d = (dst ? dst[i] : i) + dst_off;
   if (f >= n_fields) {
-    if (panel) copy_panel_part(S, s, d, f - n_fields);
+    if (panel) copy_panel_part(S, s, d, f - n_fields, panel);
     return;
   }
   if ((fields[f].cls & skip_mask) || (only_cls >= 0 && fields[f].cls != only_cls)) return;
@@ -425,12 +414,12 @@
 }
 void drlgx_launch_copy(const DrlgxField *fields_dev, int n_fields, hipStream_t st, int n, const int32_t *src,
                        const int32_t *dst, int src_off, int dst_off, int skip_mask, const int *cnt, const DrlgxState *panel,
-                       int only_cls) {
+                       int only_cls, int panel_mode) {
   if (n <= 0) return;
   const bool with_panel = panel && panel->jc;
   const dim3 cgrid(n_fields + (with_panel ? kCopySplit : 0), n);
   hipLaunchKernelGGL(k_copy_instances, cgrid, dim3(256), 0, st, fields_dev, n_fields, src, dst,
-                     src_off, dst_off, skip_mask, only_cls, cnt, with_panel ? *panel : DrlgxState{}, with_panel ? 1 : 0);
+                     src_off, dst_off, skip_mask, only_cls, cnt, with_panel ? *panel : DrlgxState{}, with_panel ? panel_mode : 0);
 }
 void drlgx_launch_fetch_pack(const DrlgxState &S, hipStream_t st, const void *src, size_t bytes, void *out) {
   const size_t head = drlgx_fetch_head_bytes(S.n_envs);
diff --git a/drl_graph_exploration_amd/csrc/k_slam_arrow.hip b/drl_graph_exploration_amd/csrc/k_slam_arrow.hip
--- a/drl_graph_exploration_amd/csrc/k_slam_arrow.hip
+++ b/drl_graph_exploration_amd/csrc/k_slam_arrow.hip
@@ -1013,6 +1013,7 @@
   extern __shared__ __attribute__((aligned(16))) unsigned char smem_raw[];
   const int tid = drlgx_tid();
   const int bi = drlgx_bid();
+  inc_settle(S, sel);
   if (!sel.on(bi)) return;
   if (S.prof && tid == 0 && bi < 448) S.prof[128 + 2 * bi] = wall_clock64();
   if (inc_stage<ISNT>(S, sel, lds_bytes, 0)) {
diff --git a/drl_graph_exploration_amd/csrc/k_step.hip b/drl_graph_exploration_amd/csrc/k_step.hip
--- a/drl_graph_exploration_amd/csrc/k_step.hip
+++ b/drl_graph_exploration_amd/csrc/k_step.hip
@@ -35,6 +35,7 @@
   bool pre = false, accepted = false, inc_try = false;
   double od3[3] = {0, 0, 0};
   int P0 = 0, L0 = 0, M0 = 0, isam = 0, pan_L0 = -1, pan_M0 = -1;
+  const double *pan_src = nullptr;
   ksim::SimPre spre;
   spre.have = tid < 64 && !sel.simlog && sel.on(bi);
   if (sel.on(bi)) {
@@ -44,7 +45,8 @@
     int meta0 = 0, meta1 = 0;
     if (S.jc) {
       const int4 mv = *reinterpret_cast<const int4 *>(kslam::inc_meta(S, inst));
-      meta0 = mv.x & 0x7fffffff;
+      meta0 = mv.x & ~kPanelInSrc;
+      if ((mv.x & kPanelInSrc) && sel.vm_from >= 0) pan_src = S.jc + (size_t)(sel.vm_from + bi) * S.jc_stride;
       meta1 = mv.y;
       pan_L0 = mv.z;
       pan_M0 = mv.w;
@@ -57,6 +59,10 @@
     const int Lb = min(S.L_max, L0 + 48), Mb = min(S.M_max, M0 + 48);
     pre = accepted && !inc_try && (3 * (P0 + 1) + 1 + 15) / 16 <= kslam::kDenseTiles && kslam::SlamCtx::big_fits(sim_bytes, lds_bytes, P0 + 1, Lb, Mb);
     if (pre) ctx.setup<true>(S, step_smem, sim_bytes, lds_bytes, inst, P0 + 1, Lb, Mb);
+  }
+  if (!inc_try) {
+    kslam::inc_settle(S, sel);
+    pan_src = nullptr;
   }
   if (tid == 0) {
     sub_cnt[0] = 0;
@@ -79,8 +85,8 @@
     bool inc_lds = false;
     if (kslam::inc_plan(S, sel.base + bi, P0 + 1, lds_bytes, sim_bytes, ix, inc_lds, pc, pan_L0, pan_M0)) {
       const kslam::SubBarrier sb{sub_cnt, kslam::kThreads / 64 - 1, 0};
-      if (inc_lds) kslam::inc_pre<true, true>(S, ix, tid, od3, sb);
-      else kslam::inc_pre<false, true>(S, ix, tid, od3, sb);
+      if (inc_lds) kslam::inc_pre<true, true>(S, ix, tid, od3, sb, pan_src);
+      else kslam::inc_pre<false, true>(S, ix, tid, od3, sb, pan_src);
     }
   }
   __syncthreads();
@@ -99,11 +105,12 @@
     bool inc_lds = false;
     if (kslam::inc_plan(S, sel.base + bi, P0 + 1, lds_bytes, sim_bytes, ix, inc_lds, pc, pan_L0, pan_M0)) {
       double *hp = hand ? reinterpret_cast<double *>(step_smem) : nullptr;
-      inc_done = inc_lds ? kslam::inc_post<true, 0>(S, ix, sub_cnt[2], sub_cnt[3], box, tid, hp, pc)
-                         : kslam::inc_post<false, 0>(S, ix, sub_cnt[2], sub_cnt[3], box, tid, hp, pc);
+      inc_done = inc_lds ? kslam::inc_post<true, 0>(S, ix, sub_cnt[2], sub_cnt[3], box, tid, hp, pc, pan_src)
+                         : kslam::inc_post<false, 0>(S, ix, sub_cnt[2], sub_cnt[3], box, tid, hp, pc, pan_src);
       if (inc_done) lm_lds = ix.thl;
       else __syncthreads();
     }
+    if (!inc_done) kslam::inc_settle(S, sel);
   }
   if (!inc_done)
     kslam::slam_finish<FT>(S, sel, lds_bytes, sim_bytes, ctx, pre, sub_cnt + 1, hand ? reinterpret_cast<double *>(step_smem) : nullptr, &lm_lds, box, pc);
diff --git a/drl_graph_exploration_amd/engine.py b/drl_graph_exploration_amd/engine.py
--- a/drl_graph_exploration_amd/engine.py
+++ b/drl_graph_exploration_amd/engine.py
@@ -478,6 +478,19 @@
         self._chk(self.L.drlgx_inc_stats_host(self.h, out, 1 if reset else 0))
         return int(out[0]), int(out[1])
 
+    def panel(self, inst):
+        meta = np.zeros(4, dtype=np.int32)
+        ipt, dpt = C.POINTER(C.c_int32), C.POINTER(C.c_double)
+        self._chk(self.L.drlgx_debug_panel_host(self.h, inst, meta.ctypes.data_as(ipt), None, 0))
+        if meta[0] != 1:
+            return meta, None
+        body = np.zeros((3 * meta[1] + 2 * meta[2], 3 + 2 * meta[2]))
+        self._chk(self.L.drlgx_debug_panel_host(self.h, inst, meta.ctypes.data_as(ipt), body.ctypes.data_as(dpt), body.size))
+        return meta, body
+
+    def snapshot_instance(self, slot, env):
+        return 2 * self.n_envs + self.n_rollouts + slot * self.n_envs + env
+
     def timing_enable(self, on=True):
         self._chk(self.L.drlgx_timing_enable(self.h, int(on)))
 
diff --git a/include/drlgx.h b/include/drlgx.h
--- a/include/drlgx.h
+++ b/include/drlgx.h
@@ -166,6 +166,7 @@
 int drlgx_debug_disc_cells_bound(double radius_cells);
 
 int drlgx_inc_stats_host(drlgx_engine *e, int64_t out[2], int reset);
+int drlgx_debug_panel_host(drlgx_engine *e, int inst, int32_t meta[4], double *panel, size_t panel_cap);
 
 
 size_t drlgx_gcn_workspace_bytes(int n_nodes, int n_edges, int hidden, int out_dim);
```
